# andrewjong/SwapNet

Hardware: AMD Instinct MI355X
Metric: images/sec full G+D step, warp-stage 256x256 bs=32/GPU (higher is better)
Workload: dtype f32; 1 GPU; warp-stage G+D optimize_parameters step, 256x256, bs 32/GPU, fp32 storage and accumulation, GEMM products on the 16-bit MFMA pipe from operand splits: forward / input-gradient GEMMs as 2 fp16 planes of amax-scaled operands (22 of 24 mantissa bits, 3 of 4 terms, the dropped one below 2^-22), weight-gradient GEMMs in the same two-plane form, train mode (dropout 0.5), WarpModule 137.6M + PatchGAN 2.8; step_form=eager launches, global_batch=32, parallelism=dp1

## Files before the change

### include/swapnet_hip.h

```cpp
#ifndef SWAPNET_HIP_H
#define SWAPNET_HIP_H

#include <stddef.h>
#include <stdint.h>

#ifdef __cplusplus
extern "C" {
#endif

typedef struct swn_ctx swn_ctx;
typedef struct swn_model swn_model;

int swn_abi_version(void);
const char* swn_last_error(void);
int swn_is_device_build(void);

int swn_ctx_create(int device, void* hip_stream, int create_stream, size_t workspace_bytes, swn_ctx** out);
int swn_ctx_destroy(swn_ctx* ctx);
int swn_ctx_set_overlap(swn_ctx* ctx, int on);
int swn_ctx_set_patchgan_layers(swn_ctx* ctx, int n_layers);
int swn_ctx_set_patchgan_norm(swn_ctx* ctx, int kind);
int swn_ctx_sync(swn_ctx* ctx);
int swn_ctx_bytes_allocated(swn_ctx* ctx, size_t* out);

int swn_prof_enable(int on);
int swn_prof_reset(void);
int swn_prof_report(char* buf, int len);
int swn_probe_mfma(swn_ctx* ctx, int zeros, int iters, float* out4);
int swn_route_trace(int on);
int swn_route_report(char* buf, int len);
int swn_slot_audit(int on);

int swn_warp_model_create(swn_ctx* ctx, int batch, int height, int width, int is_train, float dropout,
                          swn_model** out);
int swn_texture_model_create(swn_ctx* ctx, int batch, int height, int width, int is_train, int num_roi,
                             swn_model** out);
int swn_warp_model_create_ex(swn_ctx* ctx, int batch, int height, int width, int is_train, float dropout,
                             int body_channels, int cloth_channels, swn_model** out);
int swn_texture_model_create_ex(swn_ctx* ctx, int batch, int height, int width, int is_train, int num_roi,
                                int cloth_channels, swn_model** out);
int swn_texture_model_create_netG(swn_ctx* ctx, int batch, int height, int width, int is_train, int num_roi,
                                  int cloth_channels, int netG, swn_model** out);
int swn_model_create_shared(swn_model* sharer, int batch, int height, int width, swn_model** out);
int swn_model_destroy(swn_model* m);

typedef struct swn_hyper {
  float lr, d_lr, weight_decay, d_weight_decay, b1, b2;
  float lambda_gan, lambda_ce, lambda_l1, lambda_content, lambda_style;
  int gan_mode;
  int warp_mode_ce;
  float grad_scale;
  float d_b1, d_b2;
  int gp_mode;
  float lambda_gp;
} swn_hyper;
int swn_model_set_hyper(swn_model* m, const swn_hyper* h);

int swn_model_param_count(swn_model* m, int net, int* out);
int swn_model_param_info(swn_model* m, int net, int index, char* name, int name_len, int shape[4], int* ndim);
int swn_model_param_set(swn_model* m, int net, int which, const char* name, const float* dev_src);
int swn_model_param_get(swn_model* m, int net, int which, const char* name, float* dev_dst);
int swn_model_optim_step_get(swn_model* m, int net, int* step);
int swn_model_optim_step_set(swn_model* m, int net, int step);
int swn_model_set_optimizer(swn_model* m, int net, int kind, float final_lr, float base_lr, float gamma);

int swn_model_set_input(swn_model* m, int slot, const float* dev_nchw, int n, int c, int h, int w);
int swn_model_set_input_labels(swn_model* m, int slot, const int32_t* dev_labels, int n, int h, int w);
int swn_model_set_input_texture_batch(swn_model* m, const uint8_t* img, int b, int hs, int ws, const uint8_t* labels, int hl, int wl,
                                      const float* rois_raw, int r, const float* sample, const float* mean3, const float* std3,
                                      int x_min, int y_min);
int swn_model_set_input_texture_sources(swn_model* m, const uint8_t* src, size_t src_bytes, const int64_t* geom_host, int b, int hs, int ws,
                                        const uint8_t* labels, int hl, int wl, const float* rois_raw, int r, const float* sample,
                                        const float* mean3, const float* std3, int x_min, int y_min);
int swn_model_set_input_warp_batch(swn_model* m, const uint8_t* body, int b, int hb, int wb, const uint8_t* in_labels,
                                   const uint8_t* tgt_labels, int hl, int wl, const double* maps, int nmaps, const float* mean3,
                                   const float* std3, int load_size, int x_min, int y_min);
int swn_model_set_input_warp_batch_ex(swn_model* m, const uint8_t* body, int b, int hb, int wb, const uint8_t* in_labels,
                                      const uint8_t* tgt_labels, int hl, int wl, const double* maps, int nmaps, const float* mean3,
                                      const float* std3, int load_size, int x_min, int y_min, int flags);
int swn_model_get_output(swn_model* m, int slot, float* dev_nchw);
int swn_model_get_tap(swn_model* m, int net, const char* name, float* dev_nchw, int shape[4]);

int swn_model_get_tap_grad(swn_model* m, int net, const char* name, float* dev_nchw, int shape[4]);

int swn_model_dropout_sites(swn_model* m, int net, int* count);
int swn_model_act_sites(swn_model* m, int net, int* count);
int swn_model_act_pattern(swn_model* m, int net, int site, uint8_t* dev_nchw, int shape[4], int* kind);
int swn_model_dropout_mask(swn_model* m, int net, int site, uint64_t dropout_seed, float* dev_nchw, int shape[4],
                           float* p);

typedef struct swn_pipeline swn_pipeline;
int swn_pipeline_create(swn_model* warp, swn_model* texture, swn_pipeline** out);
int swn_pipeline_destroy(swn_pipeline* p);
int swn_pipeline_run(swn_pipeline* p, int use_graph, int* graph_replayed);
int swn_pipeline_labels(swn_pipeline* p, int32_t** dev_labels);
int swn_pipeline_enable_images(swn_pipeline* p, const float* body_mean3, const float* body_std3, const float* tex_mean3,
                               const float* tex_std3, const uint8_t* colours, int width, int reference_quirk);
int swn_pipeline_images(swn_pipeline* p, uint8_t** dev, int* k);
int swn_pipeline_enable_png(swn_pipeline* p, int rows_per_chunk);
int swn_pipeline_png(swn_pipeline* p, uint8_t** streams, uint32_t** sizes, size_t* stride, int* k);

int swn_model_set_style_context(swn_model* m, const float* all_out_nchw, const float* all_tgt_nchw, int n_total, int n0);
int swn_model_set_gp_random(swn_model* m, const float* alpha_dev, const float* beta_nchw_dev);
int swn_model_discriminate(swn_model* m, const float* x_nchw, float* pred_nchw);
// ... 12 lines not shown
int swn_model_backward_G_part(swn_model* m, float label_real, int part, size_t* ready_off, size_t* ready_count);
int swn_model_optimizer_step(swn_model* m, int net);
int swn_model_optimizer_step_range(swn_model* m, int net, size_t off, size_t count, int first);
int swn_model_step(swn_model* m, const float labels[3], int training, uint64_t dropout_seed);
typedef int (*swn_allreduce_fn)(const void* sendbuf, void* recvbuf, size_t count, int dtype, int op, void* comm, void* stream);
int swn_ctx_attach_comm(swn_ctx* ctx, swn_allreduce_fn fn, void* comm, int world_size);
int swn_model_step_dp(swn_model* m, const float labels[3], int training, uint64_t dropout_seed, int after_forward);
int swn_model_step_captured(swn_model* m, const float labels[3], int training, uint64_t dropout_seed);
int swn_model_get_losses(swn_model* m, float* host_out, int n);

int swn_model_grad_arena(swn_model* m, int net, float** dev_ptr, size_t* count);
int swn_model_weight_arena(swn_model* m, int net, float** dev_ptr, size_t* count);
int swn_model_arena(swn_model* m, int net, int which, float** dev_ptr, size_t* count);

int swn_op_roi_align(swn_ctx* ctx, const float* tex, int b, int c, int h, int w, const float* rois, int r,
                     int ph, int pw, float* out);
int swn_op_roi_align_indices(swn_ctx* ctx, const float* rois, int k, int h, int w, int ph, int pw, int32_t* idx,
                             uint8_t* valid);
int swn_op_decode_labels(swn_ctx* ctx, const float* x, int b, int c, int h, int w, uint8_t* rgb);
int swn_op_image_u8(swn_ctx* ctx, const float* x, int b, int c, int h, int w, const int32_t* labels, int source, const float* rows,
                    int scale_each, int range, const float* rois, int r, const uint8_t* colours, int width, uint8_t* out);
int swn_op_png_encode(swn_ctx* ctx, const uint8_t* img, int n, int h, int w, int rows_per_chunk, uint8_t* streams, size_t stream_stride,
                      uint32_t* sizes);
int swn_png_stream_bound(int h, int w, int rows_per_chunk, size_t* out);
int swn_op_argmax_labels(swn_ctx* ctx, const float* x, int b, int c, int h, int w, int32_t* labels);
int swn_op_labels_to_onehot(swn_ctx* ctx, const int32_t* labels, int b, int c, int h, int w, float* out);
int swn_op_conv(swn_ctx* ctx, int kind, int transposed, int what, int naive, float* x, int n, int ci, int h, int w,
                float* wgt, int co, const float* bias, int act, float* y);
int swn_op_conv_produced(swn_ctx* ctx, int kind, int transposed, int what, int naive, float* x, int n, int ci, int h, int w,
                         float* wgt, int co, const float* bias, int act, float* y, int pre, int post, float* x_out, float* x_slot,
                         float* y_slot, float* z_slot, float* dy_out, float* dy_slot, int* kscale_out);
int swn_op_instance_norm_act(swn_ctx* ctx, const float* x, int n, int c, int h, int w, int act, float* y);
int swn_op_instance_norm_act_bwd(swn_ctx* ctx, const float* x, const float* dy, int n, int c, int h, int w, int act,
                                 float* dx);
int swn_op_batch_norm_act(swn_ctx* ctx, const float* x, int n, int c, int h, int w, int groups, int act, int training,
                          const float* weight, const float* bias, float* running_mean, float* running_var,
                          int64_t* num_batches_tracked, float* y, float* save_stats);
int swn_op_batch_norm_act_bwd(swn_ctx* ctx, const float* x, const float* dy, int n, int c, int h, int w, int groups, int act,
                              const float* weight, const float* bias, float* dx, float* dweight, float* dbias);
int swn_op_batch_norm_act_dropout(swn_ctx* ctx, const float* x, const float* dy, int n, int c, int h, int w, int act, float p,
                                  uint64_t seed, const float* weight, const float* bias, float* y, float* mask, float* dx,
                                  float* dweight, float* dbias);
int swn_op_norm_act_time(swn_ctx* ctx, int kind, int what, const float* x, const float* dy, int n, int c, int h, int w, int groups,
                         int act, int warmup, int iters, float* ms_out);
int swn_op_affine_gather(swn_ctx* ctx, const float* src, float* dst, int b, int c, int h, int w, const double* maps,
                         int nmaps);
int swn_op_chain_resample(swn_ctx* ctx, const float* src, float* dst, int b, int c, int h, int w, const double* maps,
                          int nmaps);
int swn_op_texture_batch(swn_ctx* ctx, const uint8_t* img, int b, int hs, int ws, const uint8_t* labels, int hl, int wl,
                         const float* rois_raw, int r, const float* sample, const float* mean3, const float* std3, int x_min,
                         int y_min, int h, int w, int cloth_channels, float* in_nchw, float* tgt_nchw, float* cloths_nchw,
                         float* rois_out);
int swn_op_resize_u8(swn_ctx* ctx, const uint8_t* src, size_t src_bytes, const int64_t* geom_host, int b, int hs, int ws, uint8_t* dst);
int swn_op_warp_batch(swn_ctx* ctx, const uint8_t* body, int b, int hb, int wb, const uint8_t* in_labels, const uint8_t* tgt_labels, int hl,
                      int wl, const double* maps, int nmaps, const float* mean3, const float* std3, int load_size, int x_min, int y_min,
                      int h, int w, int cloth_channels, float* bodys_nchw, float* input_cloths_nchw, float* target_cloths_nchw);
int swn_op_warp_batch_ex(swn_ctx* ctx, const uint8_t* body, int b, int hb, int wb, const uint8_t* in_labels, const uint8_t* tgt_labels, int hl,
                         int wl, const double* maps, int nmaps, const float* mean3, const float* std3, int load_size, int x_min, int y_min,
                         int h, int w, int cloth_channels, float* bodys_nchw, float* input_cloths_nchw, float* target_cloths_nchw,
                         int flags);
int swn_op_gan_loss(swn_ctx* ctx, int gan_mode, const float* pred, int n, int c, int h, int w, float label,
                    int target_is_real, float grad_scale, float* loss_out, float* dpred);
int swn_op_loss(swn_ctx* ctx, int kind, const float* a_nchw, const float* b_nchw, int n, int c, int h, int w, int pad_c,
                float scale, int accumulate, int n0, int nloc, float* loss_out, float* da_nchw, float* pad_out);
int swn_op_bias_grad(swn_ctx* ctx, const float* dy_nchw, int n, int c, int h, int w, int pad_c, float* db);
int swn_op_norm_act_dropout(swn_ctx* ctx, const float* x, const float* dy, int n, int c, int h, int w, int norm, int act,
                            float p, uint64_t seed, float* y, float* mask, float* dx);
int swn_op_norm_act_bwd2(swn_ctx* ctx, const float* x, const float* gy, const float* u, int n, int c, int h, int w, int act,
                         float* uy, float* ax);
int swn_op_batch_norm_act_bwd2(swn_ctx* ctx, const float* x, const float* gy, const float* u, const float* gamma, const float* beta,
                               int n, int c, int h, int w, int act, float* uy, float* ax, float* dgamma);
int swn_op_norm_act(swn_ctx* ctx, const float* x, const float* dy, const float* residual, int n, int c, int h, int w, int norm,
                    int act, float drop_p, uint64_t seed, int seed_on_device, uint64_t salt, const double* partial_in,
                    int partial_chunks, const int* lead_pad, int want_colsum, float* y, float* stats, float* y_slot, float* dx,
                    float* dx_slot, double* colsum, int* colsum_emitted, float* db, float* y_buf, float* dx_buf);
int swn_op_elementwise(swn_ctx* ctx, int op, const float* a, const float* b, int n, int c, int h, int w, int act, int accumulate,
                       float alpha, float shift, const int* lead_pad, float* out, float* slot, float* out_buf);
int swn_op_resample(swn_ctx* ctx, int op, const float* a, const float* b, int n, int c, int h, int w, int factor, int accumulate,
                    const int* lead_pad, float* out, float* slot, uint8_t* pattern, float* out_buf);
int swn_op_conv_views(swn_ctx* ctx, int kind, int transposed, int what, int naive, float* x, int n, int ci, int h, int w, float* wgt,
                      int co, const float* bias, int act, float* y, const int* views, const int32_t* cimap, int cimap_len,
                      int x_is_input, int dgrad_C, int operand_slots, const float* dx_old, const int* pre_range, float* y_fwd,
                      float* y_slot, float* dw_rows, float* x_buf, float* xg_buf, float* y_buf, float* yg_buf);
int swn_op_adamw(swn_ctx* ctx, float* p, const float* g, float* m, float* v, size_t n, float lr, float b1, float b2,
                 float eps, float wd, int step);
int swn_op_adabound(swn_ctx* ctx, float* p, const float* g, float* m, float* v, size_t n, float lr, float b1, float b2,
                    float eps, float wd, float final_lr, float base_lr, float gamma, int step);

#ifdef __cplusplus
}
#endif
#endif
```

### swapnet_amd/_C.py

```python
import ctypes as C
import os

_HERE = os.path.dirname(os.path.abspath(__file__))
LIB_PATH = os.path.join(_HERE, "csrc", "libswapnet_hip.so")

LOSS_NAMES = ("D", "D_real", "D_fake", "G", "G_gan", "G_ce", "G_l1", "G_content", "G_style", "D_gp")


class SwnHyper(C.Structure):
    _fields_ = [(n, C.c_float) for n in ("lr", "d_lr", "weight_decay", "d_weight_decay", "b1", "b2",
                                         "lambda_gan", "lambda_ce", "lambda_l1", "lambda_content",
                                         "lambda_style")] + [("gan_mode", C.c_int), ("warp_mode_ce", C.c_int), ("grad_scale", C.c_float),
                                                                           ("d_b1", C.c_float), ("d_b2", C.c_float),
                                                                           ("gp_mode", C.c_int), ("lambda_gp", C.c_float)]


class SwapnetHipError(RuntimeError):
    pass


_vp, _fp, _i, _f = C.c_void_p, C.c_void_p, C.c_int, C.c_float

_PROTOS = {
    "swn_abi_version": ([], _i),
    "swn_is_device_build": ([], _i),
    "swn_ctx_create": ([_i, _vp, _i, C.c_size_t, C.POINTER(_vp)], _i),
    "swn_ctx_destroy": ([_vp], _i),
    "swn_ctx_sync": ([_vp], _i),
    "swn_ctx_set_overlap": ([_vp, _i], _i),
    "swn_ctx_set_patchgan_layers": ([_vp, _i], _i),
    "swn_ctx_set_patchgan_norm": ([_vp, _i], _i),
    "swn_ctx_bytes_allocated": ([_vp, C.POINTER(C.c_size_t)], _i),
    "swn_prof_enable": ([_i], _i),
    "swn_prof_reset": ([], _i),
    "swn_prof_report": ([C.c_char_p, _i], _i),
    "swn_probe_mfma": ([_vp, _i, _i, C.POINTER(C.c_float)], _i),
    "swn_route_trace": ([_i], _i),
    "swn_route_report": ([C.c_char_p, _i], _i),
    "swn_slot_audit": ([_i], _i),
    "swn_warp_model_create": ([_vp, _i, _i, _i, _i, _f, C.POINTER(_vp)], _i),
    "swn_texture_model_create": ([_vp, _i, _i, _i, _i, _i, C.POINTER(_vp)], _i),
    "swn_warp_model_create_ex": ([_vp, _i, _i, _i, _i, _f, _i, _i, C.POINTER(_vp)], _i),
    "swn_texture_model_create_ex": ([_vp, _i, _i, _i, _i, _i, _i, C.POINTER(_vp)], _i),
    "swn_texture_model_create_netG": ([_vp, _i, _i, _i, _i, _i, _i, _i, C.POINTER(_vp)], _i),
    "swn_model_create_shared": ([_vp, _i, _i, _i, C.POINTER(_vp)], _i),
    "swn_model_destroy": ([_vp], _i),
    "swn_model_set_hyper": ([_vp, C.POINTER(SwnHyper)], _i),
    "swn_model_param_count": ([_vp, _i, C.POINTER(_i)], _i),
    "swn_model_param_info": ([_vp, _i, _i, C.c_char_p, _i, C.POINTER(_i * 4), C.POINTER(_i)], _i),
    "swn_model_param_set": ([_vp, _i, _i, C.c_char_p, _fp], _i),
    "swn_model_param_get": ([_vp, _i, _i, C.c_char_p, _fp], _i),
    "swn_model_optim_step_get": ([_vp, _i, C.POINTER(_i)], _i),
    "swn_model_optim_step_set": ([_vp, _i, _i], _i),
    "swn_model_set_optimizer": ([_vp, _i, _i, _f, _f, _f], _i),
    "swn_model_set_input": ([_vp, _i, _fp, _i, _i, _i, _i], _i),
    "swn_model_set_input_labels": ([_vp, _i, _vp, _i, _i, _i], _i),
    "swn_model_set_input_texture_batch": ([_vp, _vp, _i, _i, _i, _vp, _i, _i, _fp, _i, _fp, C.POINTER(_f), C.POINTER(_f), _i, _i], _i),
    "swn_model_set_input_texture_sources": ([_vp, _vp, C.c_size_t, _vp, _i, _i, _i, _vp, _i, _i, _fp, _i, _fp, C.POINTER(_f), C.POINTER(_f),
                                             _i, _i], _i),
    "swn_model_set_input_warp_batch": ([_vp, _vp, _i, _i, _i, _vp, _vp, _i, _i, _vp, _i, C.POINTER(_f), C.POINTER(_f), _i, _i, _i], _i),
    "swn_model_set_input_warp_batch_ex": ([_vp, _vp, _i, _i, _i, _vp, _vp, _i, _i, _vp, _i, C.POINTER(_f), C.POINTER(_f), _i, _i, _i, _i], _i),
    "swn_model_get_output": ([_vp, _i, _fp], _i),
    "swn_model_get_tap": ([_vp, _i, C.c_char_p, _fp, C.POINTER(_i * 4)], _i),
    "swn_model_get_tap_grad": ([_vp, _i, C.c_char_p, _fp, C.POINTER(_i * 4)], _i),
    "swn_model_dropout_sites": ([_vp, _i, C.POINTER(_i)], _i),
    "swn_model_act_sites": ([_vp, _i, C.POINTER(_i)], _i),
    "swn_model_act_pattern": ([_vp, _i, _i, _vp, C.POINTER(_i * 4), C.POINTER(_i)], _i),
    "swn_model_dropout_mask": ([_vp, _i, _i, C.c_uint64, _fp, C.POINTER(_i * 4), C.POINTER(_f)], _i),
    "swn_pipeline_create": ([_vp, _vp, C.POINTER(_vp)], _i),
    "swn_pipeline_destroy": ([_vp], _i),
    "swn_pipeline_run": ([_vp, _i, C.POINTER(_i)], _i),
    "swn_pipeline_labels": ([_vp, C.POINTER(_vp)], _i),
    "swn_pipeline_enable_images": ([_vp, C.POINTER(_f), C.POINTER(_f), C.POINTER(_f), C.POINTER(_f), C.POINTER(C.c_uint8), _i, _i], _i),
    "swn_pipeline_images": ([_vp, C.POINTER(_vp), C.POINTER(_i)], _i),
    "swn_pipeline_enable_png": ([_vp, _i], _i),
    "swn_pipeline_png": ([_vp, C.POINTER(_vp), C.POINTER(_vp), C.POINTER(C.c_size_t), C.POINTER(_i)], _i),
    "swn_op_png_encode": ([_vp, _vp, _i, _i, _i, _i, _vp, C.c_size_t, _vp], _i),
    "swn_png_stream_bound": ([_i, _i, _i, C.POINTER(C.c_size_t)], _i),
    "swn_op_image_u8": ([_vp, _fp, _i, _i, _i, _i, _vp, _i, _fp, _i, _i, _fp, _i, _vp, _i, _vp], _i),
    "swn_model_set_style_context": ([_vp, _fp, _fp, _i, _i], _i),
    "swn_model_set_gp_random": ([_vp, _fp, _fp], _i),
    "swn_model_discriminate": ([_vp, _fp, _fp], _i),
    "swn_model_set_discriminate_mode": ([_vp, _i], _i),
    "swn_model_buffer_count": ([_vp, _i, C.POINTER(_i)], _i),
    "swn_model_buffer_info": ([_vp, _i, _i, C.c_char_p, _i, C.POINTER(_i), C.POINTER(_i)], _i),
    "swn_model_buffer_set": ([_vp, _i, C.c_char_p, _vp], _i),
    "swn_model_buffer_get": ([_vp, _i, C.c_char_p, _vp], _i),
    "swn_model_perceptual": ([_vp, _fp, _fp, _i, _fp, _f, _f, _fp], _i),
    "swn_model_forward": ([_vp, _i, C.c_uint64], _i),
    "swn_model_backward_D": ([_vp, _f, _f], _i),
    "swn_model_backward_G": ([_vp, _f], _i),
    "swn_model_backward_G_parts": ([_vp, C.POINTER(C.c_int)], _i),
    "swn_model_backward_G_part": ([_vp, _f, _i, C.POINTER(C.c_size_t), C.POINTER(C.c_size_t)], _i),
    "swn_model_optimizer_step": ([_vp, _i], _i),
    "swn_model_optimizer_step_range": ([_vp, _i, C.c_size_t, C.c_size_t, _i], _i),
    "swn_model_step": ([_vp, C.POINTER(_f * 3), _i, C.c_uint64], _i),
    "swn_model_step_captured": ([_vp, C.POINTER(_f * 3), _i, C.c_uint64], _i),
    "swn_model_step_dp": ([_vp, C.POINTER(_f * 3), _i, C.c_uint64, _i], _i),
    "swn_ctx_attach_comm": ([_vp, _vp, _vp, _i], _i),
    "swn_model_get_losses": ([_vp, C.POINTER(_f), _i], _i),
    "swn_model_grad_arena": ([_vp, _i, C.POINTER(_vp), C.POINTER(C.c_size_t)], _i),
    "swn_model_weight_arena": ([_vp, _i, C.POINTER(_vp), C.POINTER(C.c_size_t)], _i),
    "swn_model_arena": ([_vp, _i, _i, C.POINTER(_vp), C.POINTER(C.c_size_t)], _i),
    "swn_op_roi_align": ([_vp, _fp, _i, _i, _i, _i, _fp, _i, _i, _i, _fp], _i),
    "swn_op_roi_align_indices": ([_vp, _fp, _i, _i, _i, _i, _i, _vp, _vp], _i),
    "swn_op_decode_labels": ([_vp, _fp, _i, _i, _i, _i, _vp], _i),
    "swn_op_argmax_labels": ([_vp, _fp, _i, _i, _i, _i, _vp], _i),
    "swn_op_labels_to_onehot": ([_vp, _vp, _i, _i, _i, _i, _fp], _i),
    "swn_op_conv": ([_vp, _i, _i, _i, _i, _fp, _i, _i, _i, _i, _fp, _i, _fp, _i, _fp], _i),
    "swn_op_conv_produced": ([_vp, _i, _i, _i, _i, _fp, _i, _i, _i, _i, _fp, _i, _fp, _i, _fp, _i, _i, _fp, _fp, _fp, _fp, _fp, _fp, _vp], _i),
    "swn_op_instance_norm_act": ([_vp, _fp, _i, _i, _i, _i, _i, _fp], _i),
    "swn_op_instance_norm_act_bwd": ([_vp, _fp, _fp, _i, _i, _i, _i, _i, _fp], _i),
    "swn_op_batch_norm_act": ([_vp, _fp, _i, _i, _i, _i, _i, _i, _i, _fp, _fp, _fp, _fp, _vp, _fp, _fp], _i),
    "swn_op_batch_norm_act_bwd": ([_vp, _fp, _fp, _i, _i, _i, _i, _i, _i, _fp, _fp, _fp, _fp, _fp], _i),
    "swn_op_batch_norm_act_dropout": ([_vp, _fp, _fp, _i, _i, _i, _i, _i, _f, C.c_uint64, _fp, _fp, _fp, _fp, _fp, _fp, _fp], _i),
    "swn_op_norm_act_time": ([_vp, _i, _i, _fp, _fp, _i, _i, _i, _i, _i, _i, _i, _i, C.POINTER(C.c_float)], _i),
    "swn_op_affine_gather": ([_vp, _fp, _fp, _i, _i, _i, _i, _vp, _i], _i),
    "swn_op_texture_batch": ([_vp, _vp, _i, _i, _i, _vp, _i, _i, _fp, _i, _fp, C.POINTER(_f), C.POINTER(_f), _i, _i, _i, _i, _i,
                             _fp, _fp, _fp, _fp], _i),
    "swn_op_resize_u8": ([_vp, _vp, C.c_size_t, _vp, _i, _i, _i, _vp], _i),
    "swn_op_warp_batch": ([_vp, _vp, _i, _i, _i, _vp, _vp, _i, _i, _vp, _i, C.POINTER(_f), C.POINTER(_f), _i, _i, _i, _i, _i, _i,
                          _fp, _fp, _fp], _i),
    "swn_op_warp_batch_ex": ([_vp, _vp, _i, _i, _i, _vp, _vp, _i, _i, _vp, _i, C.POINTER(_f), C.POINTER(_f), _i, _i, _i, _i, _i, _i,
                             _fp, _fp, _fp, _i], _i),
    "swn_op_chain_resample": ([_vp, _fp, _fp, _i, _i, _i, _i, _vp, _i], _i),
    "swn_op_gan_loss": ([_vp, _i, _fp, _i, _i, _i, _i, _f, _i, _f, _fp, _fp], _i),
    "swn_op_loss": ([_vp, _i, _fp, _fp, _i, _i, _i, _i, _i, _f, _i, _i, _i, _fp, _fp, _fp], _i),
    "swn_op_bias_grad": ([_vp, _fp, _i, _i, _i, _i, _i, _fp], _i),
    "swn_op_norm_act": ([_vp, _fp, _fp, _fp, _i, _i, _i, _i, _i, _i, _f, C.c_uint64, _i, C.c_uint64, _vp, _i, C.POINTER(_i), _i,
                         _fp, _fp, _fp, _fp, _fp, _vp, C.POINTER(_i), _fp, _fp, _fp], _i),
    "swn_op_elementwise": ([_vp, _i, _fp, _fp, _i, _i, _i, _i, _i, _i, _f, _f, C.POINTER(_i), _fp, _fp, _fp], _i),
    "swn_op_resample": ([_vp, _i, _fp, _fp, _i, _i, _i, _i, _i, _i, C.POINTER(_i), _fp, _fp, _vp, _fp], _i),
    "swn_op_conv_views": ([_vp, _i, _i, _i, _i, _fp, _i, _i, _i, _i, _fp, _i, _fp, _i, _fp, C.POINTER(_i), C.POINTER(C.c_int32), _i, _i, _i, _i,
                           _fp, C.POINTER(_i), _fp, _fp, _fp, _fp, _fp, _fp, _fp], _i),
    "swn_op_norm_act_bwd2": ([_vp, _fp, _fp, _fp, _i, _i, _i, _i, _i, _fp, _fp], _i),
    "swn_op_batch_norm_act_bwd2": ([_vp, _fp, _fp, _fp, _fp, _fp, _i, _i, _i, _i, _i, _fp, _fp, _fp], _i),
    "swn_op_norm_act_dropout": ([_vp, _fp, _fp, _i, _i, _i, _i, _i, _i, _f, C.c_uint64, _fp, _fp, _fp], _i),
    "swn_op_adamw": ([_vp, _fp, _fp, _fp, _fp, C.c_size_t, _f, _f, _f, _f, _f, _i], _i),
    "swn_op_adabound": ([_vp, _fp, _fp, _fp, _fp, C.c_size_t, _f, _f, _f, _f, _f, _f, _f, _f, _i], _i),
}


class Lib:

    def __init__(self, path=None):
        self.path = path or LIB_PATH
        if not os.path.exists(self.path):
            raise SwapnetHipError(
                f"{self.path} not found: build it with `python -m swapnet_amd.build` "
                "(hipcc --offload-arch=gfx950).  swapnet_amd has no CPU fallback.")
        import torch
        self.dll = C.CDLL(self.path)
        self.dll.swn_last_error.restype = C.c_char_p
        self.dll.swn_last_error.argtypes = []
        for name, (args, res) in _PROTOS.items():
            fn = getattr(self.dll, name)
            fn.argtypes = args
            fn.restype = res
        self.is_device = bool(self.dll.swn_is_device_build())

    def last_error(self):
        return (self.dll.swn_last_error() or b"").decode()

    def call(self, name, *args):
        rc = getattr(self.dll, name)(*args)
        if rc != 0:
            msg = self.last_error()
            if "not implemented" in msg or "not recognized" in msg:
                raise NotImplementedError(msg)
            if rc == 1:
                raise ValueError(msg)
            raise SwapnetHipError(msg)
        return rc

    @staticmethod
    def exported_symbols():
        return ["swn_last_error"] + list(_PROTOS)


_default = None


def lib():
    global _default
    if _default is None:
        _default = Lib()
        if not _default.is_device:
            raise SwapnetHipError("libswapnet_hip.so is not a device build")
    return _default


def ptr(t):
    if t is None:
        return None
    assert t.is_contiguous(), "tensor must be contiguous"
    return C.c_void_p(t.data_ptr())
```

### swapnet_amd/csrc/capi.cpp

```cpp
#include <algorithm>
#include <cstring>
#include <memory>
#include <string>
#include <vector>

#include "../../include/swapnet_hip.h"
#include <cstdlib>

#include "engine.h"

using namespace swn;

struct CtxBox {
  std::unique_ptr<Ctx> c;
  void* owned_stream = nullptr;
  ~CtxBox() { c.reset(); if (owned_stream) stream_destroy(owned_stream); }
};
struct swn_ctx {
  std::shared_ptr<CtxBox> box;
  Ctx* c = nullptr;
};
struct swn_model {
  std::shared_ptr<CtxBox> keep;
  std::shared_ptr<Model> sharer;
// ... 3 lines not shown
  float dropout = 0.5f;
};
struct swn_pipeline {
  std::shared_ptr<CtxBox> keep;
  std::unique_ptr<Pipeline> p;
};

static thread_local std::string g_err;

template <typename F>
static int guard(F f) {
  try {
    f();
    return 0;
  } catch (const Error& e) {
    g_err = e.what();
    return e.code ? e.code : 1;
  } catch (const std::exception& e) {
    g_err = e.what();
    return 1;
  } catch (...) {
    g_err = "unknown error";
    return 1;
  }
}
#define REQUIRE(cond, msg) \
  do { if (!(cond)) throw Error(1, msg); } while (0)

extern "C" {

int swn_abi_version(void) { return 9; }
const char* swn_last_error(void) { return g_err.c_str(); }
int swn_is_device_build(void) { return is_device_build(); }

int swn_ctx_create(int device, void* hip_stream, int create_stream, size_t workspace_bytes, swn_ctx** out) {
  return guard([&] {
    REQUIRE(out, "swn_ctx_create: out is NULL");
    auto h = std::make_unique<swn_ctx>();
    h->box = std::make_shared<CtxBox>();
    void* st = hip_stream;
    if (create_stream) { st = stream_create(device); h->box->owned_stream = st; }
    else device_check(device);
    if (workspace_bytes < (size_t)64 << 20) workspace_bytes = (size_t)64 << 20;
    h->box->c = std::make_unique<Ctx>(st, workspace_bytes);
    h->c = h->box->c.get();
    h->c->device_index = device;
    if (env_on(getenv("SWN_OVERLAP"))) h->c->enable_side(device);
    *out = h.release();
  });
}
int swn_ctx_destroy(swn_ctx* ctx) {
  return guard([&] {
    if (!ctx) return;
    delete ctx;
  });
}
int swn_ctx_set_overlap(swn_ctx* ctx, int on) {
  return guard([&] {
    REQUIRE(ctx, "ctx is NULL");
    ctx->c->join_side();
    stream_sync(ctx->c->s);
    ctx->c->side_enabled = on != 0;
  });
}
int swn_ctx_attach_comm(swn_ctx* ctx, swn_allreduce_fn fn, void* comm, int world_size) {
  return guard([&] {
    REQUIRE(ctx, "ctx is NULL");
    ctx->c->join_side();
    ctx->c->attach_comm(reinterpret_cast<Ctx::AllReduceFn>(fn), comm, fn ? world_size : 1);
  });
}
int swn_ctx_set_patchgan_layers(swn_ctx* ctx, int n_layers) {
  return guard([&] {
    REQUIRE(ctx, "ctx is NULL");
    REQUIRE(n_layers >= 0 && n_layers <= 5, "n_layers_D must be in [1, 5], or 0 for the 1x1 PixelDiscriminator");
    ctx->c->patchgan_layers = n_layers;
  });
}
int swn_ctx_set_patchgan_norm(swn_ctx* ctx, int kind) {
  return guard([&] {
    REQUIRE(ctx, "ctx is NULL");
    REQUIRE(kind >= 0 && kind <= 2, "normalization layer is not found (0 instance, 1 batch, 2 none)");
    ctx->c->patchgan_norm = kind;
  });
}
int swn_ctx_sync(swn_ctx* ctx) {
  return guard([&] { REQUIRE(ctx, "ctx is NULL"); stream_sync(ctx->c->s); });
}
int swn_ctx_bytes_allocated(swn_ctx* ctx, size_t* out) {
  return guard([&] { REQUIRE(ctx && out, "NULL argument"); *out = ctx->c->bytes_allocated; });
}

int swn_prof_enable(int on) { return guard([&] { prof_enable(on); }); }
int swn_prof_reset(void) { return guard([&] { prof_reset(); }); }
int swn_prof_report(char* buf, int len) { return prof_report(buf, len); }
int swn_probe_mfma(swn_ctx* ctx, int zeros, int iters, float* out4) {
  return guard([&] {
    REQUIRE(ctx && out4, "swn_probe_mfma: NULL argument");
    REQUIRE(iters >= 1 && iters <= (1 << 20), "swn_probe_mfma: iters out of range");
    probe_mfma(ctx->c->s, zeros, iters, out4);
  });
}
int swn_route_trace(int on) { return guard([&] { route_enable(on); }); }
int swn_route_report(char* buf, int len) { return route_report(buf, len); }
int swn_slot_audit(int on) { return guard([&] { slot_audit(on); }); }
struct AuditSuspend {
  int was = slot_audit_on();
  AuditSuspend() { slot_audit(0); }
  ~AuditSuspend() { slot_audit(was); }
};

int swn_warp_model_create_ex(swn_ctx* ctx, int batch, int height, int width, int is_train, float dropout,
                             int body_channels, int cloth_channels, swn_model** out) {
  return guard([&] {
    REQUIRE(ctx && out, "NULL argument");
    REQUIRE(batch > 0 && height > 0 && width > 0, "bad shape");
    auto h = std::make_unique<swn_model>();
    h->keep = ctx->box;
    h->m.reset(create_warp_model(*ctx->c, batch, height, width, is_train != 0, dropout, body_channels, cloth_channels));
    h->kind = 0; h->is_train = is_train != 0; h->dropout = dropout; h->body_channels = body_channels; h->cloth_channels = cloth_channels;
    h->patchgan_layers = ctx->c->patchgan_layers; h->patchgan_norm = ctx->c->patchgan_norm;
    *out = h.release();
  });
}
int swn_warp_model_create(swn_ctx* ctx, int batch, int height, int width, int is_train, float dropout,
                          swn_model** out) {
  return swn_warp_model_create_ex(ctx, batch, height, width, is_train, dropout, 3, 19, out);
}
int swn_texture_model_create_netG(swn_ctx* ctx, int batch, int height, int width, int is_train, int num_roi,
                                  int cloth_channels, int netG, swn_model** out) {
  return guard([&] {
    REQUIRE(ctx && out, "NULL argument");
    auto h = std::make_unique<swn_model>();
    h->keep = ctx->box;
    h->m.reset(create_texture_model(*ctx->c, batch, height, width, is_train != 0, num_roi, cloth_channels, nullptr, netG));
    h->kind = 1; h->is_train = is_train != 0; h->num_roi = num_roi; h->cloth_channels = cloth_channels;
    h->patchgan_layers = ctx->c->patchgan_layers; h->netG = netG;
    *out = h.release();
  });
}
int swn_texture_model_create_ex(swn_ctx* ctx, int batch, int height, int width, int is_train, int num_roi,
                                int cloth_channels, swn_model** out) {
  return swn_texture_model_create_netG(ctx, batch, height, width, is_train, num_roi, cloth_channels, NETG_SWAPNET, out);
}
int swn_texture_model_create(swn_ctx* ctx, int batch, int height, int width, int is_train, int num_roi,
                             swn_model** out) {
  return swn_texture_model_create_ex(ctx, batch, height, width, is_train, num_roi, 19, out);
}
int swn_model_create_shared(swn_model* sharer, int batch, int height, int width, swn_model** out) {
  return guard([&] {
    REQUIRE(sharer && out, "NULL argument");
    REQUIRE(batch > 0 && height > 0 && width > 0, "bad shape");
    std::shared_ptr<Model> root = sharer->sharer ? sharer->sharer : sharer->m;
    Ctx& c = *root->ctx;
    auto h = std::make_unique<swn_model>();
    h->keep = sharer->keep;
    h->sharer = root;
    h->kind = sharer->kind; h->is_train = sharer->is_train; h->dropout = sharer->dropout; h->num_roi = sharer->num_roi;
    h->body_channels = sharer->body_channels; h->cloth_channels = sharer->cloth_channels; h->patchgan_layers = sharer->patchgan_layers;
    h->patchgan_norm = sharer->patchgan_norm; h->netG = sharer->netG;
    const int layers_was = c.patchgan_layers, norm_was = c.patchgan_norm;
    c.patchgan_layers = sharer->patchgan_layers; c.patchgan_norm = sharer->patchgan_norm;
    try {
      if (h->kind == 0)
        h->m.reset(create_warp_model(c, batch, height, width, h->is_train != 0, h->dropout, h->body_channels, h->cloth_channels, root.get()));
      else
// ... 1220 lines not shown
    if (yg_buf) nhwc_to_nchw(s, yo.parent.g, yg_buf, yo.parent.g.C);
    stream_sync(s);
  });
}
int swn_op_norm_act_bwd2(swn_ctx* ctx, const float* x, const float* gy, const float* u, int n, int c, int h, int w, int act,
                         float* uy, float* ax) {
  return guard([&] {
    REQUIRE(ctx && x && gy && u && uy && ax && c % 4 == 0, "bad argument (C must be a multiple of 4)");
    Ctx tmp(ctx->c->s);
    ParamArena A; Net net(tmp, A);
    Var xv = net.alloc_var(n, h, w, c, true), yv = net.alloc_var(n, h, w, c, true), uv = net.alloc_var(n, h, w, c, true);
    net.norm_act(xv, yv, true, act, 0.f);
    net.finalize({});
    nchw_to_nhwc(tmp.s, x, n, c, h, w, xv.v);
    nchw_to_nhwc(tmp.s, gy, n, c, h, w, yv.g);
    nchw_to_nhwc(tmp.s, u, n, c, h, w, uv.v);
    net.forward();
    NormActBwd2Args b2;
    b2.u = uv.v; b2.gy = yv.g; b2.x = xv.v; b2.stats = net.last_stats; b2.uy = uv.g; b2.ax = xv.g; b2.act = act;
    norm_act_bwd2(tmp.s, b2);
    nhwc_to_nchw(tmp.s, uv.g, uy, c);
    nhwc_to_nchw(tmp.s, xv.g, ax, c);
    stream_sync(tmp.s);
  });
}
int swn_op_batch_norm_act_bwd2(swn_ctx* ctx, const float* x, const float* gy, const float* u, const float* gamma, const float* beta,
                               int n, int c, int h, int w, int act, float* uy, float* ax, float* dgamma) {
  return guard([&] {
    REQUIRE(ctx && x && gy && u && gamma && beta && uy && ax && dgamma && c % 4 == 0, "bad argument (C must be a multiple of 4)");
    REQUIRE(n > 0 && c > 0 && h > 0 && w > 0, "bad shape");
    Ctx tmp(ctx->c->s);
    ParamArena A; Net net(tmp, A);
    Var xv = net.alloc_var(n, h, w, c, true), yv = net.alloc_var(n, h, w, c, true), uv = net.alloc_var(n, h, w, c, true);
    float* par = static_cast<float*>(tmp.alloc((size_t)7 * c * sizeof(float)));
    float *gd = par, *bd = par + c, *stats = par + 2 * c, *fold = par + 4 * c, *dg = par + 6 * c;
    dev_copy(tmp.s, gd, gamma, c * sizeof(float));
    dev_copy(tmp.s, bd, beta, c * sizeof(float));
    nchw_to_nhwc(tmp.s, x, n, c, h, w, xv.v);
    nchw_to_nhwc(tmp.s, gy, n, c, h, w, yv.g);
    nchw_to_nhwc(tmp.s, u, n, c, h, w, uv.v);
    BatchNormArgs f;
    f.x = xv.v; f.y = yv.v; f.gamma = gd; f.beta = bd; f.stats = stats; f.fold = fold; f.act = act;
    batch_norm_fwd(tmp.s, f);
    BatchNormBwd2Args b2;
    b2.u = uv.v; b2.gy = yv.g; b2.x = xv.v; b2.stats = stats; b2.fold = fold; b2.gamma = gd;
    b2.uy = uv.g; b2.ax = xv.g; b2.dgamma = dg; b2.act = act;
    batch_norm_bwd2(tmp.s, b2);
    nhwc_to_nchw(tmp.s, uv.g, uy, c);
    nhwc_to_nchw(tmp.s, xv.g, ax, c);
    dev_copy(tmp.s, dgamma, dg, c * sizeof(float));
    stream_sync(tmp.s);
  });
}
int swn_op_norm_act_dropout(swn_ctx* ctx, const float* x, const float* dy, int n, int c, int h, int w, int norm, int act,
                            float p, uint64_t seed, float* y, float* mask, float* dx) {
  return guard([&] {
    REQUIRE(ctx && x && y && c % 4 == 0, "bad argument (C must be a multiple of 4)");
    REQUIRE(p >= 0.f && p < 1.f, "dropout probability must be in [0, 1)");
    Ctx tmp(ctx->c->s);
    ParamArena A; Net net(tmp, A);
    Var xv = net.alloc_var(n, h, w, c, true), yv = net.alloc_var(n, h, w, c, true);
    net.norm_act(xv, yv, norm != 0, act, p);
    net.finalize({});
    net.training = true; net.seed = seed;
    nchw_to_nhwc(tmp.s, x, n, c, h, w, xv.v);
    net.forward();
    nhwc_to_nchw(tmp.s, yv.v, y, c);
    if (mask) {
      if (p > 0.f) {
        const Net::DropSite& d = net.drop_sites.at(0);
        dropout_mask(tmp.s, d.N, d.H, d.W, d.C, d.p, Net::drop_seed(seed, d.salt), mask);
      } else {
        REQUIRE(false, "mask requested with p == 0");
      }
    }
    if (dy && dx) {
      nchw_to_nhwc(tmp.s, dy, n, c, h, w, yv.g);
      net.backward(false, true);
      nhwc_to_nchw(tmp.s, xv.g, dx, c);
    }
    stream_sync(tmp.s);
  });
}
int swn_op_adamw(swn_ctx* ctx, float* p, const float* g, float* m, float* v, size_t n, float lr, float b1, float b2,
                 float eps, float wd, int step) {
  return guard([&] {
    REQUIRE(ctx && p && g && m && v, "NULL argument");
    AdamWArgs a{p, g, m, v, n, lr, b1, b2, eps, wd, step};
    adamw_step(ctx->c->s, a);
    stream_sync(ctx->c->s);
  });
}
int swn_op_adabound(swn_ctx* ctx, float* p, const float* g, float* m, float* v, size_t n, float lr, float b1, float b2,
                    float eps, float wd, float final_lr, float base_lr, float gamma, int step) {
  return guard([&] {
    REQUIRE(ctx && p && g && m && v, "NULL argument");
    REQUIRE(step >= 1 && base_lr > 0.f && gamma > 0.f, "AdaBound needs step >= 1, base_lr > 0, gamma > 0");
    if (!is_device_build()) throw Error(1, "swn_op_adabound: AdaBound is not implemented on the host simulator (HIP kernel only)");
    AdamWArgs a{p, g, m, v, n, lr, b1, b2, eps, wd, step};
    a.kind = OPT_ADABOUND; a.final_lr = final_lr; a.base_lr = base_lr; a.gamma = gamma;
    adamw_step(ctx->c->s, a);
    stream_sync(ctx->c->s);
  });
}

}
```

### swapnet_amd/csrc/engine.cpp

```cpp
#include "engine.h"
#include "png_chunk.h"
#include <memory>

#include <algorithm>
#include <cstddef>
#include <cstdlib>
#include <cstring>
#include <map>
#include <string>
#include <vector>

namespace swn {

namespace {
int g_route = 0;
std::string g_route_label = "-";
char g_route_phase = '-';
std::vector<std::string> g_route_lines;
std::map<std::string, int> g_route_seen;
}
void route_enable(int on) {
  g_route = on;
  if (on) { g_route_lines.clear(); g_route_seen.clear(); g_route_label = "-"; g_route_phase = '-'; }
}
// ... 205 lines not shown
  dg_layout.push_back({op, off});
  return off;
}

namespace {
struct ConvGeom {
  Gather fwd;
  int Ho = 0, Wo = 0;
};
ConvGeom conv_geom(ConvKind kind, int H, int W) {
  ConvGeom c;
  Gather& g = c.fwd;
  switch (kind) {
    case CK_K4S2: g.KH = g.KW = 4; g.stride = 2; g.pad_t = g.pad_l = 1; c.Ho = H / 2; c.Wo = W / 2; break;
    case CK_K3S1_REFLECT: g.KH = g.KW = 3; g.stride = 1; g.pad_t = g.pad_l = 1; g.pad_mode = PAD_REFLECT; c.Ho = H; c.Wo = W; break;
    case CK_K3S1_ZERO: g.KH = g.KW = 3; g.stride = 1; g.pad_t = g.pad_l = 1; c.Ho = H; c.Wo = W; break;
    case CK_K4S1: g.KH = g.KW = 4; g.stride = 1; g.pad_t = g.pad_l = 1; c.Ho = H - 1; c.Wo = W - 1; break;
    case CK_K1S1: g.KH = g.KW = 1; g.stride = 1; g.pad_t = g.pad_l = 0; c.Ho = H; c.Wo = W; break;
    case CK_TAIL_UP:
      g.KH = g.KW = 4; g.stride = 1; g.pad_t = g.pad_l = 2; g.ups = 1; c.Ho = H * 2; c.Wo = W * 2; break;
  }
  g.Ho = c.Ho; g.Wo = c.Wo;
  return c;
}

struct WinoSwitches {
  bool on, s2_on;
  int minc, force_m;
};
WinoSwitches wino_switches() {
  return {env_on(getenv("SWN_WINOGRAD")), env_on(getenv("SWN_WINO_S2")), env_int(getenv("SWN_WINO_MINC"), 0), env_int(getenv("SWN_WINO_M"), 0)};
}

bool s2_wino_wanted(const WinoSwitches& sw, int Cfine, int Ccoarse, int Hc, int Wc) {
  if (!sw.on || !sw.s2_on) return false;
  const int minc = sw.minc > 0 ? sw.minc : 256;
  if (Ccoarse < minc || Cfine < 32 || Cfine % 4 || Ccoarse % 16 || Hc < 2 || Wc < 2) return false;
  if (sw.minc <= 0 && Hc * Wc < 256) return false;
  return (size_t)16 * Cfine * Ccoarse <= ((size_t)1 << 22);
}

int wino_s1_m(const WinoSwitches& sw, ConvKind kind, int Cip, int Co, int H, int W) {
  const bool is_k3 = kind == CK_K3S1_REFLECT || kind == CK_K3S1_ZERO, is_k4 = kind == CK_K4S1;
  const int wm = is_k4 ? 3 : ((sw.force_m != 2 && H % 4 == 0 && W % 4 == 0) ? 4 : 2);
  const int minc = sw.minc > 0 ? sw.minc : (wm == 2 ? 256 : 64);
  const bool wino = sw.on && Cip % 32 == 0 && Co % 32 == 0 && Cip >= minc && Co >= minc && H >= 4 && W >= 4 &&
                    ((is_k3 && H % 2 == 0 && W % 2 == 0) || is_k4);
  return wino ? wm : 0;
}

TView plane_mat(float* p, size_t T, int C) {
  TView v; v.p = p; v.N = 1; v.H = 1; v.W = (int)T; v.C = C; v.cs = C; return v;
}
struct PlaneScale { const int* pair_k = nullptr; const float* amax = nullptr; };
PlaneScale plane_scale(bool pairs, const int* k, const float* amax) { return pairs ? PlaneScale{k, nullptr} : PlaneScale{nullptr, amax}; }
struct PlanePanel { const float* w; const uint16_t* pc; int tile; size_t bs; };
ConvFwdArgs plane_gemm(float* x, float* y, size_t T, int K, int N, int Cout, int P, PlaneScale xs, PlanePanel w) {
  ConvFwdArgs g;
  g.x = plane_mat(x, T, K); g.g.Ho = 1; g.g.Wo = (int)T;
  g.w = w.w; g.Npad = N; g.Cout = Cout;
  g.y = plane_mat(y, T, N);
  g.batch = P; g.x_bs = T * K; g.w_bs = (size_t)K * N; g.y_bs = T * N;
  g.x_pair_k = xs.pair_k; g.x_amax = xs.amax;
  if (w.tile) { g.wpc = w.pc; g.wpc_bn = w.tile; g.wpc_bs = w.bs; }
  return g;
}
ConvWgradArgs plane_wgrad(float* x, float* dy, float* dw, size_t T, int K, int N, int Cout, int P, PlaneScale xs, PlaneScale dys) {
  ConvWgradArgs g;
  g.x = plane_mat(x, T, K); g.g.Ho = 1; g.g.Wo = (int)T;
  g.dy = plane_mat(dy, T, N);
  g.dw = dw; g.Npad = N; g.Cout = Cout;
  g.batch = P; g.x_bs = T * K; g.dy_bs = T * N; g.dw_bs = (size_t)K * N;
  g.x_pair_k = xs.pair_k; g.x_amax = xs.amax;
  g.dy_pair_k = dys.pair_k; g.dy_amax = dys.amax;
  return g;
}

int wino_precut_tile(int xC, int Npad) {
  const int t = conv_precut_tile(xC, Npad);
  return (t == 64 || t == 128) ? t : 0;
}
bool wino_fwd_takes_pairs(int xC, int Npad) { return wino_precut_tile(xC, Npad) != 0 && conv_fwd_takes_pairs(xC, Npad); }

bool bias_on_main() { static const bool on = env_on(getenv("SWN_BIAS_MAIN")); return on; }
}

struct Net::ConvLayer {
  const std::string& name;
  const Var &x, &y;
  ConvKind kind;
  int Ci, Co, Cip, Cop;
  int wi, bi;
  int actf;
  ConvGeom geo;
  bool x_is_input;
  int dgrad_C;
};

void Net::conv(const std::string& name, const Var& x, const Var& y, ConvKind kind, int Ci, int Co, bool bias,
               int actf, const std::vector<int32_t>* cimap, bool x_is_input, int dgrad_C) {
  const WinoSwitches sw = wino_switches();
  const int KH = kind == CK_K1S1 ? 1 : ((kind == CK_K3S1_REFLECT || kind == CK_K3S1_ZERO) ? 3 : 4);
  const ConvGeom geo = conv_geom(kind, x.v.H, x.v.W);
  if (y.v.H != geo.Ho || y.v.W != geo.Wo) throw Error(1, "conv " + name + ": output view has the wrong size");
  const int Cip = x.v.C;
  if (Ci > Cip) throw Error(1, "conv " + name + ": Ci exceeds the input view's channels");
  const int wi = arena.add_weight(name + ".weight", WK_CONV, Co, Ci, KH, KH, Cip, cimap);
  const int bi = bias ? arena.add_bias(name + ".bias", Co) : -1;
  const int Cop = round_up(Co, 4);
  if (y.v.C != Cop) throw Error(1, "conv " + name + ": output view must have round_up(Co,4) channels");
  note_act(actf, y.v);

  auto op = std::make_unique<Op>();
  op->label = name;
  op->param_off = arena.params[wi].off;
  op->reads_net_input = x_is_input;
  const ConvLayer L{name, x, y, kind, Ci, Co, Cip, Cop, wi, bi, actf, geo, x_is_input, dgrad_C};
  if (env_on(getenv("SWN_HEAD_TAPN")) && kind == CK_K4S1 && Co == 1 && Cip % 32 == 0 && actf == ACT_NONE && x.has_grad == y.has_grad)
    conv_head_tapn(L, *op);
  else if (kind == CK_K4S2 && s2_wino && !x_is_input && s2_wino_wanted(sw, Cip, Cop, y.v.H, y.v.W) && Co % 4 == 0)
    conv_wino_s2(L, *op);
  else if (kind == CK_TAIL_UP && sw.on && Cip % 32 == 0 && Cip >= (sw.minc > 0 ? sw.minc : 64) && x.v.H >= 4 && x.v.W >= 4 && Cop <= 32)
    conv_tail_wino(L, *op);
  else if (const int wm = wino_s1_m(sw, kind, Cip, Co, x.v.H, x.v.W))
    conv_wino_s1(L, wm, *op);
  else
    conv_direct(L, *op);
  ops.push_back(std::move(op));
}

void Net::conv_head_tapn(const ConvLayer& L, Op& op) {
  const Var &x = L.x, &y = L.y;
  const int Cip = L.Cip, wi = L.wi, bi = L.bi;
  ParamArena* A = &arena; Op* self = &op;
  const TView xv = x.v, yv = y.v;
  const size_t wt_off = reserve_dg(self, (size_t)Cip * 16), wt2_off = reserve_dg(self, (size_t)16 * Cip);
  const size_t dwt_off = reserve_dg(self, (size_t)Cip * 16);
  note_writer(y.vbase, false);
  Var Z = alloc_var(xv.N, xv.H, xv.W, 16, false);
  const TView zv = Z.v, ygv = y.g, xgv = x.g;
  const bool has_grad = y.has_grad;
  op.repack = [=](Net& n) {
    const ParamDesc& wd = A->params[wi];
    head_pack(n.ctx.s, wd.ws, A->w + wd.off, n.dg + wt_off, n.dg + wt2_off);
  };
  op.fwd = [=](Net& n) {
    n.need(self);
    ConvFwdArgs a;
    a.x = xv; a.g.Ho = xv.H; a.g.Wo = xv.W;
    a.w = n.dg + wt_off; a.Npad = 16; a.Cout = 16; a.y = zv;
    conv_fwd(n.ctx.s, a);
    head_gather(n.ctx.s, zv, bi >= 0 ? A->w + A->params[bi].off : nullptr, yv);
  };
  if (has_grad) op.grad_targets.push_back(x);
  op.bwd = [=](Net& n, Op& me, bool wgrad, bool igrad) {
    if (!has_grad) return;
    const ParamDesc& wd = A->params[wi];
    head_scatter(n.ctx.s, ygv, zv);
    if (wgrad) {
      Stream& sw = n.wgrad_stream();
      ConvWgradArgs wa;
      wa.x = xv; wa.g.Ho = xv.H; wa.g.Wo = xv.W; wa.dy = zv;
      wa.dw = n.dg + dwt_off; wa.Npad = 16; wa.Cout = 16;
      conv_wgrad(sw, wa);
      head_unpack_grad(sw, wd.ws, n.dg + dwt_off, A->g + wd.off);
      if (bi >= 0) n.bias_grad_of(sw, ygv, A->g + A->params[bi].off);
    }
    if (me.reads_net_input && !igrad) return;
    ConvFwdArgs d;
    d.x = zv; d.g.Ho = xv.H; d.g.Wo = xv.W;
    d.w = n.dg + wt2_off; d.Npad = Cip; d.Cout = Cip; d.y = xgv; d.accumulate = me.acc.empty() ? 0 : me.acc[0];
    conv_fwd(n.ctx.s, d);
  };
}

void Net::conv_wino_s2(const ConvLayer& L, Op& op) {
  const Var &x = L.x, &y = L.y;
  const int Co = L.Co, Cip = L.Cip, Cop = L.Cop, wi = L.wi, bi = L.bi, actf = L.actf;
  ParamArena* A = &arena; Op* self = &op;
  const TView xv = x.v, yv = y.v;
  const int sP = 25, sTh = ceil_div(y.v.H, 4), sTw = ceil_div(y.v.W, 4), CV = 4 * Cip;
  const size_t sT = (size_t)x.v.N * sTh * sTw;
  const bool want_dx = x.has_grad && y.has_grad;
  const size_t uf_off = reserve_dg(self, (size_t)sP * CV * Cop);
  const size_t ut_off = want_dx ? reserve_dg(self, (size_t)sP * Cop * CV) : 0;
  float* keepV = (keep_wino_inputs && y.has_grad) ? static_cast<float*>(ctx.alloc(sP * sT * CV * sizeof(float))) : nullptr;
  wsV_need = std::max(wsV_need, sP * sT * (size_t)std::max(CV, Cop));
  wsM_need = std::max(wsM_need, sP * sT * (size_t)std::max(CV, Cop));
  wsU_need = std::max(wsU_need, (size_t)sP * CV * Cop);
  const int pcf = conv_precut_tile(CV, Cop), pct = want_dx ? conv_precut_tile(Cop, CV) : 0;
  const size_t pcf_bs = pcf ? conv_precut_elems(CV, Cop, pcf) : 0, pct_bs = pct ? conv_precut_elems(Cop, CV, pct) : 0;
  const size_t pcf_off = pcf ? reserve_dgp(pcf_bs * sP) : 0, pct_off = pct ? reserve_dgp(pct_bs * sP) : 0;
  const size_t slV = reserve_slot(), slD = reserve_slot();
  note_writer(y.vbase, false);
  const bool pairV_ok = conv_fwd_takes_pairs(CV, Cop) && (!y.has_grad || conv_wgrad_takes_pairs(sT, CV, Cop));
  const bool pairD_ok = conv_wgrad_takes_pairs(sT, CV, Cop) && (!(x.has_grad && y.has_grad) || conv_fwd_takes_pairs(Cop, CV));
  const size_t kV = reserve_k(), kD = reserve_k();
  const float* xbase = x.vbase; const float* ygbase = y.gbase;
  float* keepdM = (y.has_grad && want_dx && share_dy()) ? static_cast<float*>(ctx.alloc(sP * sT * Cop * sizeof(float))) : nullptr;
  op.repack = [=](Net& n) {
    const ParamDesc& wd = A->params[wi];
    const float* wmax = nullptr;
    wino_s2_filter_transform(n.ctx.s, wd.ws, 0, A->w + wd.off, n.dg + uf_off);
    if (pcf) conv_precut(n.ctx.s, n.dg + uf_off, CV, Cop, pcf, sP, (size_t)CV * Cop, n.dgp + pcf_off, &wmax);
    if (want_dx) {
      wino_s2_filter_transform(n.ctx.s, wd.ws, 1, A->w + wd.off, n.dg + ut_off);
      if (pct) conv_precut(n.ctx.s, n.dg + ut_off, Cop, CV, pct, sP, (size_t)Cop * CV, n.dgp + pct_off, &wmax);
    }
  };
  op.fwd = [=](Net& n) {
    n.need(self);
    float* V = keepV ? keepV : n.wsV;
    const float* xin = pairV_ok ? n.slot_if_complete(xbase) : nullptr;
    wino_s2_input_transform(n.ctx.s, xv, sTh, sTw, V, n.amax + slV, xin, n.kscale + kV);
    conv_fwd(n.ctx.s, plane_gemm(V, n.wsM, sT, CV, Cop, Co, sP, plane_scale(xin != nullptr, n.kscale + kV, n.amax + slV),
                                 {n.dg + uf_off, n.dgp + pcf_off, pcf, pcf_bs}));
    wino_output_transform(n.ctx.s, 4, 2, n.wsM, Cop, sTh, sTw, bi >= 0 ? A->w + A->params[bi].off : nullptr, actf, yv, Co, 0);
  };
  Var scratch;
  if (y.has_grad && actf != ACT_NONE) scratch = alloc_var(yv.N, yv.H, yv.W, Cop, false);
  if (want_dx) op.grad_targets.push_back(x);
  const TView ygv = y.g, xgv = x.g, scr = scratch.v;
  const bool has_ygrad = y.has_grad;
  op.bwd = [=](Net& n, Op& me, bool wgrad, bool igrad) {
    if (!has_ygrad) return;
    TView dY = ygv;
    if (actf != ACT_NONE) { act_bwd(n.ctx.s, ygv, yv, scr, actf, 0); dY = scr; }
    const ParamDesc& wd = A->params[wi];
    const bool dx_now = want_dx && !(me.reads_net_input && !igrad);
    const bool shared = keepdM && wgrad && dx_now;
    const float* xin = pairV_ok ? n.slot_if_complete(xbase) : nullptr;
    const float* din = (pairD_ok && actf == ACT_NONE) ? n.slot_if_complete(ygbase) : nullptr;
    const PlaneScale dMs = plane_scale(din != nullptr, n.kscale + kD, n.amax + slD);
    if (shared) wino_dy_transform(n.ctx.s, 4, 2, dY, sTh, sTw, keepdM, n.amax + slD, din, n.kscale + kD);
    if (wgrad) {
      Stream& sw = n.wgrad_stream();
      float* V = keepV ? keepV : n.wsV;
      float* dM = shared ? keepdM : n.wgrad_planes(sw);
      if (!keepV) wino_s2_input_transform(sw, xv, sTh, sTw, V, n.amax + slV, xin, n.kscale + kV);
      if (!shared) wino_dy_transform(sw, 4, 2, dY, sTh, sTw, dM, n.amax + slD, din, n.kscale + kD);
      conv_wgrad(sw, plane_wgrad(V, dM, n.wsU, sT, CV, Cop, Co, sP, plane_scale(xin != nullptr, n.kscale + kV, n.amax + slV), dMs));
      wino_s2_filter_grad(sw, wd.ws, n.wsU, A->g + wd.off);
      if (bi >= 0) n.bias_grad_of(sw, dY, A->g + A->params[bi].off);
    }
    if (!dx_now) return;
    float* dMx = shared ? keepdM : n.wsV;
    if (!shared) wino_dy_transform(n.ctx.s, 4, 2, dY, sTh, sTw, dMx, n.amax + slD, din, n.kscale + kD);
    conv_fwd(n.ctx.s, plane_gemm(dMx, n.wsM, sT, Cop, CV, CV, sP, dMs, {n.dg + ut_off, n.dgp + pct_off, pct, pct_bs}));
    wino_s2_input_adjoint(n.ctx.s, n.wsM, Cip, sTh, sTw, xgv, nullptr, me.acc.empty() ? 0 : me.acc[0]);
  };
}

void Net::conv_tail_wino(const ConvLayer& L, Op& op) {
  const Var &x = L.x, &y = L.y;
  const int Co = L.Co, Cip = L.Cip, Cop = L.Cop, wi = L.wi, bi = L.bi, actf = L.actf;
  ParamArena* A = &arena; Op* self = &op;
  const TView xv = x.v, yv = y.v;
  const ParamDesc wd0 = arena.params[wi];
  const int tP = 36, tTh = ceil_div(x.v.H, 4), tTw = ceil_div(x.v.W, 4), N4 = 4 * Cop;
  const size_t tT = (size_t)x.v.N * tTh * tTw;
  const size_t fe = tail_fold_offset(wd0.ws, 4);
  const size_t fold_off = reserve_dg(self, fe), dfold_off = reserve_dg(self, fe);
  const size_t tu_off = reserve_dg(self, (size_t)tP * Cip * N4);
  float* keepV = (keep_wino_inputs && y.has_grad) ? static_cast<float*>(ctx.alloc(tP * tT * Cip * sizeof(float))) : nullptr;
  wsV_need = std::max(wsV_need, tP * tT * (size_t)std::max(Cip, N4));
  wsM_need = std::max(wsM_need, tP * tT * (size_t)std::max(Cip, N4));
  wsU_need = std::max(wsU_need, (size_t)tP * Cip * N4);
  const int pcu = conv_precut_tile(Cip, N4);
  const size_t pcu_bs = pcu ? conv_precut_elems(Cip, N4, pcu) : 0, pcu_off = pcu ? reserve_dgp(pcu_bs * tP) : 0;
  const size_t slV = reserve_slot(), slD = reserve_slot();
  note_writer(y.vbase, false);
  const bool pairV_ok = conv_fwd_takes_pairs(Cip, N4) && (!y.has_grad || conv_wgrad_takes_pairs(tT, Cip, N4));
  const bool pairD_ok = conv_wgrad_takes_pairs(tT, Cip, N4);
  const size_t kV = reserve_k(), kD = reserve_k();
  const float* xbase = x.vbase;
  const bool want_dx = x.has_grad && y.has_grad;
  const int CopD = (actf != ACT_NONE && want_dx && conv_precut_tile(32, Cip) == 192) ? 32 : Cop;
  const size_t dg_off = want_dx ? reserve_dg(self, dgrad_elems(wd0.ws, 3, CopD, Cip)) : 0;
  const int pc_d = want_dx ? conv_precut_tile(CopD, Cip) : 0;
  const size_t pcd_bs = pc_d ? conv_precut_elems(25 * CopD, Cip, pc_d) : 0, pcd_off = pc_d ? reserve_dgp(pcd_bs) : 0;
  op.repack = [=](Net& n) {
    const ParamDesc& wd = A->params[wi];
    tail_fold_weights(n.ctx.s, wd.ws, A->w + wd.off, n.dg + fold_off);
    tailw_filter_transform(n.ctx.s, wd.ws, n.dg + fold_off, n.dg + tu_off);
    if (pcu) conv_precut(n.ctx.s, n.dg + tu_off, Cip, N4, pcu, tP, (size_t)Cip * N4, n.dgp + pcu_off);
    if (want_dx) {
      repack_dgrad(n.ctx.s, wd.ws, 3, CopD, Cip, A->w + wd.off, n.dg + dg_off);
      if (pc_d) conv_precut(n.ctx.s, n.dg + dg_off, 25 * CopD, Cip, pc_d, 1, 0, n.dgp + pcd_off);
    }
  };
  op.fwd = [=](Net& n) {
    n.need(self);
    float* V = keepV ? keepV : n.wsV;
    const float* xin = pairV_ok ? n.slot_if_complete(xbase) : nullptr;
    wino_input_transform(n.ctx.s, 4, 3, xv, 1, PAD_ZERO, tTh, tTw, V, n.amax + slV, xin, n.kscale + kV);
    conv_fwd(n.ctx.s, plane_gemm(V, n.wsM, tT, Cip, N4, N4, tP, plane_scale(xin != nullptr, n.kscale + kV, n.amax + slV),
                                 {n.dg + tu_off, n.dgp + pcu_off, pcu, pcu_bs}));
    tailw_output_transform(n.ctx.s, n.wsM, tTh, tTw, Cop, bi >= 0 ? A->w + A->params[bi].off : nullptr, actf, yv, Co);
  };
  Var scratch;
  if (y.has_grad && actf != ACT_NONE) scratch = alloc_var(yv.N, yv.H, yv.W, CopD, false);
  if (want_dx) op.grad_targets.push_back(x);
  const TView ygv = y.g, xgv = x.g, scr = CopD != Cop ? scratch.v.slice(0, Cop) : scratch.v, scr_full = scratch.v;
  const bool has_ygrad = y.has_grad;
  const size_t scrSlot = (y.has_grad && actf != ACT_NONE) ? note_writer(scratch.v.p, true) : 0;
  op.bwd = [=](Net& n, Op& me, bool wgrad, bool igrad) {
    if (!has_ygrad) return;
    TView dY = ygv;
    const float* dy_slot = nullptr;
    if (actf != ACT_NONE) { act_bwd(n.ctx.s, ygv, yv, scr, actf, 0, n.amax + scrSlot); dY = scr; dy_slot = n.amax + scrSlot; }
    const ParamDesc& wd = A->params[wi];
    if (wgrad) {
      Stream& sw = n.wgrad_stream();
      float* V = keepV ? keepV : n.wsV;
      float* dM = n.wgrad_planes(sw);
      const float* xin = pairV_ok ? n.slot_if_complete(xbase) : nullptr;
      const float* din = pairD_ok ? dy_slot : nullptr;
      if (!keepV) wino_input_transform(sw, 4, 3, xv, 1, PAD_ZERO, tTh, tTw, V, n.amax + slV, xin, n.kscale + kV);
      tailw_dy_transform(sw, dY, tTh, tTw, Cop, dM, n.amax + slD, din, n.kscale + kD);
      conv_wgrad(sw, plane_wgrad(V, dM, n.wsU, tT, Cip, N4, N4, tP, plane_scale(xin != nullptr, n.kscale + kV, n.amax + slV),
                                 plane_scale(din != nullptr, n.kscale + kD, n.amax + slD)));
      tailw_filter_grad(sw, wd.ws, n.wsU, n.dg + dfold_off);
      tail_unfold_wgrad(sw, wd.ws, n.dg + dfold_off, A->g + wd.off);
      if (bi >= 0) n.bias_grad_of(sw, dY, A->g + A->params[bi].off);
    }
    if (!want_dx || (me.reads_net_input && !igrad)) return;
    ConvFwdArgs d;
    d.x = CopD != Cop ? scr_full : dY;
    d.g.KH = d.g.KW = 5; d.g.stride = 2; d.g.pad_t = d.g.pad_l = 1; d.g.Ho = xv.H; d.g.Wo = xv.W;
    d.w = n.dg + dg_off; d.Npad = Cip; d.Cout = Cip; d.y = xgv; d.accumulate = me.acc.empty() ? 0 : me.acc[0];
    d.x_amax = dy_slot;
// ... 205 lines not shown
        repack_dgrad(n.ctx.s, wd.ws, dg_mode, CopD, Ndg, A->w + wd.off, n.dg + dg_off);
        if (pc_d) conv_precut(n.ctx.s, n.dg + dg_off, dKp, Ndg, pc_d, dpanels, (size_t)dKp * Ndg, n.dgp + pcd_off, &wmax);
      }
      if (folded) tail_fold_weights(n.ctx.s, wd.ws, A->w + wd.off, n.dg + fold_off);
    };
  const TView ygv = y.g, xgv = narrow_dx ? x.g.slice(0, Ndg) : x.g, scr = CopD != Cop ? scratch.v.slice(0, Cop) : scratch.v, scr_full = scratch.v, dxp = dxpad.v;
  const bool has_ygrad = y.has_grad;
  const size_t scrSlot = (y.has_grad && actf != ACT_NONE) ? note_writer(scratch.v.p, true) : 0;
  const float* ygbase = y.gbase;
  op.bwd = [=](Net& n, Op& me, bool wgrad, bool igrad) {
    if (!has_ygrad) return;
    TView dY = ygv;
    const float* dy_slot = nullptr;
    if (actf != ACT_NONE) { act_bwd(n.ctx.s, ygv, yv, scr, actf, 0, n.amax + scrSlot); dY = scr; dy_slot = n.amax + scrSlot; }
    else dy_slot = n.slot_if_complete(ygbase);
    const ParamDesc& wd = A->params[wi];
    const bool dx_now = want_dx && !(me.reads_net_input && !igrad);
    if (wgrad) {
      Stream& sw = n.wgrad_stream();
      ConvWgradArgs wa;
      wa.x = xv; wa.g = gf; wa.dy = dY; wa.dw = A->g + wd.off; wa.Npad = wd.ws.Npad; wa.Cout = Co;
      wa.x_amax = n.slot_if_complete(xbase); wa.dy_amax = dy_slot;
      if (!folded) {
        conv_wgrad(sw, wa);
      } else {
        wa.x_amax = wa.dy_amax = nullptr;
        wa.g = Gather(); wa.g.KH = wa.g.KW = 3; wa.g.stride = 1; wa.g.pad_t = wa.g.pad_l = 1; wa.g.Ho = xv.H; wa.g.Wo = xv.W;
        wa.om.ymul = wa.om.xmul = 2; wa.tail4 = 1;
        wa.dw = n.dg + dfold_off;
        conv_wgrad(sw, wa);
        tail_unfold_wgrad(sw, wd.ws, n.dg + dfold_off, A->g + wd.off);
      }
      if (bi >= 0) n.bias_grad_of((!dx_now && bias_on_main()) ? n.ctx.s : sw, dY, A->g + A->params[bi].off);
    }
    if (!dx_now) return;
    const int accf = me.acc.empty() ? 0 : me.acc[0];
    ConvFwdArgs d;
    d.w = n.dg + dg_off; d.Npad = Ndg; d.Cout = Ndg;
    d.x_amax = dy_slot;
    if (pc_d) { d.wpc = n.dgp + pcd_off; d.wpc_bn = pc_d; d.wpc_bs = pcd_bs; }
    if (kind == CK_K4S2) {
      d.x = dY; d.g.KH = d.g.KW = 2; d.g.stride = 1; d.g.pad_t = 1; d.g.pad_l = 1;
      d.g.Ho = dY.H; d.g.Wo = dY.W;
      d.w_bs = (size_t)4 * Cop * Ndg;
      d.y = xgv; d.om.ymul = 2; d.om.xmul = 2; d.phases = 4; d.accumulate = accf;
      conv_fwd(n.ctx.s, d);
    } else if (kind == CK_K3S1_REFLECT) {
      d.x = dY; d.g = gd; d.y = dxp; d.accumulate = 0;
      conv_fwd(n.ctx.s, d);
      reflect_fold(n.ctx.s, dxp, xgv, accf);
    } else {
      d.x = CopD != Cop ? scr_full : dY; d.g = gd; d.y = xgv; d.accumulate = accf;
      conv_fwd(n.ctx.s, d);
    }
  };
}

void Net::convT(const std::string& name, const Var& x, const Var& y, int Co, bool bias) {
  const WinoSwitches sw = wino_switches();
  if (y.v.H != x.v.H * 2 || y.v.W != x.v.W * 2) throw Error(1, "convT " + name + ": output view has the wrong size");
  const int Cip = x.v.C, Cop = round_up(Co, 4);
  if (y.v.C != Cop) throw Error(1, "convT " + name + ": output view must have round_up(Co,4) channels");
  const int wi = arena.add_weight(name + ".weight", WK_CONVT, Co, Cip, 4, 4, Cip, nullptr);
  const int bi = bias ? arena.add_bias(name + ".bias", Co) : -1;
  auto op = std::make_unique<Op>();
  op->label = name;
  op->param_off = arena.params[wi].off;
  note_writer(y.vbase, false);
  const ConvLayer L{name, x, y, CK_K4S2, Cip, Co, Cip, Cop, wi, bi, ACT_NONE, ConvGeom(), false, 0};
  if (s2_wino && s2_wino_wanted(sw, Cop, Cip, x.v.H, x.v.W) && Co % 4 == 0) convT_wino_s2(L, *op);
  else convT_direct(L, *op);
  ops.push_back(std::move(op));
}

void Net::convT_wino_s2(const ConvLayer& L, Op& op) {
  const Var &x = L.x, &y = L.y;
  const int Cip = L.Cip, Cop = L.Cop, wi = L.wi, bi = L.bi;
  ParamArena* A = &arena; Op* self = &op;
  const TView xv = x.v, yv = y.v, ygv = y.g, xgv = x.g;
  const float* xbase = x.vbase; const float* ygbase = y.gbase;
  const int sP = 25, sTh = ceil_div(x.v.H, 4), sTw = ceil_div(x.v.W, 4), CV = 4 * Cop;
  const size_t sT = (size_t)x.v.N * sTh * sTw;
  const bool want_dx = x.has_grad && y.has_grad;
  const size_t ut_off = reserve_dg(self, (size_t)sP * Cip * CV);
  const size_t uf_off = want_dx ? reserve_dg(self, (size_t)sP * CV * Cip) : 0;
  float* keepM = (keep_wino_inputs && y.has_grad) ? static_cast<float*>(ctx.alloc(sP * sT * Cip * sizeof(float))) : nullptr;
  wsV_need = std::max(wsV_need, sP * sT * (size_t)std::max(CV, Cip));
  wsM_need = std::max(wsM_need, sP * sT * (size_t)std::max(CV, Cip));
  wsU_need = std::max(wsU_need, (size_t)sP * CV * Cip);
  const int pct = conv_precut_tile(Cip, CV), pcf = want_dx ? conv_precut_tile(CV, Cip) : 0;
  const size_t pct_bs = pct ? conv_precut_elems(Cip, CV, pct) : 0, pcf_bs = pcf ? conv_precut_elems(CV, Cip, pcf) : 0;
  const size_t pct_off = pct ? reserve_dgp(pct_bs * sP) : 0, pcf_off = pcf ? reserve_dgp(pcf_bs * sP) : 0;
  const size_t slM = reserve_slot(), slV = reserve_slot();
  const bool wg_pairs = conv_wgrad_takes_pairs(sT, CV, Cip);
  const bool pairM_ok = conv_fwd_takes_pairs(Cip, CV) && (!y.has_grad || wg_pairs);
  const bool pairV_ok = wg_pairs && (!(x.has_grad && y.has_grad) || conv_fwd_takes_pairs(CV, Cip));
  const size_t kM = reserve_k(), kVg = reserve_k();
  float* keepVg = (y.has_grad && want_dx && share_dy()) ? static_cast<float*>(ctx.alloc(sP * sT * CV * sizeof(float))) : nullptr;
  op.repack = [=](Net& n) {
    const ParamDesc& wd = A->params[wi];
    wino_s2_filter_transform(n.ctx.s, wd.ws, 1, A->w + wd.off, n.dg + ut_off);
    const float* wmax = nullptr;
    if (pct) conv_precut(n.ctx.s, n.dg + ut_off, Cip, CV, pct, sP, (size_t)Cip * CV, n.dgp + pct_off, &wmax);
    if (want_dx) {
      wino_s2_filter_transform(n.ctx.s, wd.ws, 0, A->w + wd.off, n.dg + uf_off);
      if (pcf) conv_precut(n.ctx.s, n.dg + uf_off, CV, Cip, pcf, sP, (size_t)CV * Cip, n.dgp + pcf_off, &wmax);
    }
  };
  op.fwd = [=](Net& n) {
    n.need(self);
    float* dM = keepM ? keepM : n.wsV;
    const float* xin = pairM_ok ? n.slot_if_complete(xbase) : nullptr;
    wino_dy_transform(n.ctx.s, 4, 2, xv, sTh, sTw, dM, n.amax + slM, xin, n.kscale + kM);
    conv_fwd(n.ctx.s, plane_gemm(dM, n.wsM, sT, Cip, CV, CV, sP, plane_scale(xin != nullptr, n.kscale + kM, n.amax + slM),
                                 {n.dg + ut_off, n.dgp + pct_off, pct, pct_bs}));
    wino_s2_input_adjoint(n.ctx.s, n.wsM, Cop, sTh, sTw, yv, bi >= 0 ? A->w + A->params[bi].off : nullptr, 0);
  };
  if (want_dx) op.grad_targets.push_back(x);
  const bool has_ygrad = y.has_grad;
  op.bwd = [=](Net& n, Op& me, bool wgrad, bool igrad) {
    if (!has_ygrad) return;
    const ParamDesc& wd = A->params[wi];
    const bool dx_now = want_dx && !(me.reads_net_input && !igrad);
    const bool shared = keepVg && wgrad && dx_now;
    const float* xin = pairM_ok ? n.slot_if_complete(xbase) : nullptr;
    const float* din = pairV_ok ? n.slot_if_complete(ygbase) : nullptr;
    const PlaneScale Vs = plane_scale(din != nullptr, n.kscale + kVg, n.amax + slV);
    if (shared) wino_s2_input_transform(n.ctx.s, ygv, sTh, sTw, keepVg, n.amax + slV, din, n.kscale + kVg);
    if (wgrad) {
      Stream& sw = n.wgrad_stream();
      float* V = shared ? keepVg : n.wgrad_planes(sw);
      float* dM = keepM ? keepM : n.wsV;
      if (!shared) wino_s2_input_transform(sw, ygv, sTh, sTw, V, n.amax + slV, din, n.kscale + kVg);
      if (!keepM) wino_dy_transform(sw, 4, 2, xv, sTh, sTw, dM, n.amax + slM, xin, n.kscale + kM);
      conv_wgrad(sw, plane_wgrad(V, dM, n.wsU, sT, CV, Cip, Cip, sP, Vs, plane_scale(xin != nullptr, n.kscale + kM, n.amax + slM)));
      wino_s2_filter_grad(sw, wd.ws, n.wsU, A->g + wd.off);
      if (bi >= 0) n.bias_grad_of(sw, ygv, A->g + A->params[bi].off);
    }
    if (!dx_now) return;
    float* Vx = shared ? keepVg : n.wsV;
    if (!shared) wino_s2_input_transform(n.ctx.s, ygv, sTh, sTw, Vx, n.amax + slV, din, n.kscale + kVg);
    conv_fwd(n.ctx.s, plane_gemm(Vx, n.wsM, sT, CV, Cip, Cip, sP, Vs, {n.dg + uf_off, n.dgp + pcf_off, pcf, pcf_bs}));
    wino_output_transform(n.ctx.s, 4, 2, n.wsM, Cip, sTh, sTw, nullptr, ACT_NONE, xgv, Cip, me.acc.empty() ? 0 : me.acc[0]);
  };
}

void Net::convT_direct(const ConvLayer& L, Op& op) {
  const Var &x = L.x, &y = L.y;
  const int Co = L.Co, Cip = L.Cip, Cop = L.Cop, wi = L.wi, bi = L.bi;
  ParamArena* A = &arena; Op* self = &op;
  const TView xv = x.v, yv = y.v, ygv = y.g, xgv = x.g;
  const float* xbase = x.vbase; const float* ygbase = y.gbase;
  const size_t phase_elems = (size_t)4 * Cip * round_up(Co, 4);
  const int pc_f = conv_precut_tile(Cip, Cop);
  const size_t pcf_bs = pc_f ? conv_precut_elems(4 * Cip, Cop, pc_f) : 0;
  const size_t pcf_off = pc_f ? reserve_dgp(pcf_bs * 4) : 0;
  op.fwd = [=](Net& n) {
    const ParamDesc& wd = A->params[wi];
    ConvFwdArgs f;
    if (pc_f) { n.need(self); f.wpc = n.dgp + pcf_off; f.wpc_bn = pc_f; f.wpc_bs = pcf_bs; }
    f.x = xv; f.g.KH = f.g.KW = 2; f.g.stride = 1; f.g.pad_t = 1; f.g.pad_l = 1; f.g.Ho = xv.H; f.g.Wo = xv.W;
    f.w = A->w + wd.off; f.w_bs = phase_elems; f.Npad = wd.ws.Npad;
    f.x_amax = n.slot_if_complete(xbase);
    f.bias = bi >= 0 ? A->w + A->params[bi].off : nullptr;
    f.y = yv; f.om.ymul = 2; f.om.xmul = 2; f.phases = 4; f.Cout = Co;
    conv_fwd(n.ctx.s, f);
  };
  const bool want_dx = x.has_grad && y.has_grad;
  size_t dg_off = 0, pcd_off = 0;
  const int pc_d = want_dx ? conv_precut_tile(Cop, Cip) : 0;
  if (want_dx) {
    dg_off = reserve_dg(self, dgrad_elems(arena.params[wi].ws, 2, Cop, Cip));
    if (pc_d) pcd_off = reserve_dgp(conv_precut_elems(16 * Cop, Cip, pc_d));
    op.grad_targets.push_back(x);
  }
  if (want_dx || pc_f)
    op.repack = [=](Net& n) {
      const ParamDesc& wd = A->params[wi];
      const float* wmax = nullptr;
      if (pc_f) conv_precut(n.ctx.s, A->w + wd.off, 4 * Cip, Cop, pc_f, 4, phase_elems, n.dgp + pcf_off, &wmax);
      if (want_dx) {
        repack_dgrad(n.ctx.s, wd.ws, 2, Cop, Cip, A->w + wd.off, n.dg + dg_off);
        if (pc_d) conv_precut(n.ctx.s, n.dg + dg_off, 16 * Cop, Cip, pc_d, 1, 0, n.dgp + pcd_off, &wmax);
      }
    };
  const bool has_ygrad = y.has_grad;
  op.bwd = [=](Net& n, Op& me, bool wgrad, bool igrad) {
    if (!has_ygrad) return;
    const ParamDesc& wd = A->params[wi];
    if (wgrad) {
      ConvWgradArgs wa;
      wa.x = xv; wa.g.KH = wa.g.KW = 2; wa.g.stride = 1; wa.g.pad_t = 1; wa.g.pad_l = 1;
      wa.g.Ho = xv.H; wa.g.Wo = xv.W;
      wa.dy = ygv; wa.om.ymul = 2; wa.om.xmul = 2; wa.phases = 4;
      wa.dw = A->g + wd.off; wa.dw_bs = phase_elems; wa.Npad = wd.ws.Npad; wa.Cout = Co;
      wa.x_amax = n.slot_if_complete(xbase); wa.dy_amax = n.slot_if_complete(ygbase);
      Stream& sw = n.wgrad_stream();
      conv_wgrad(sw, wa);
      if (bi >= 0) n.bias_grad_of(sw, ygv, A->g + A->params[bi].off);
    }
    if (!want_dx || (me.reads_net_input && !igrad)) return;
    ConvFwdArgs d;
    d.x = ygv; d.g.KH = d.g.KW = 4; d.g.stride = 2; d.g.pad_t = d.g.pad_l = 1; d.g.Ho = xv.H; d.g.Wo = xv.W;
    d.w = n.dg + dg_off; d.Npad = Cip; d.Cout = Cip; d.y = xgv; d.accumulate = me.acc.empty() ? 0 : me.acc[0];
    d.x_amax = n.slot_if_complete(ygbase);
    if (pc_d) { d.wpc = n.dgp + pcd_off; d.wpc_bn = pc_d; }
    conv_fwd(n.ctx.s, d);
  };
}

void Net::norm_act(const Var& raw, const Var& y, bool norm, int actf, float drop_p, const Var* residual) {
  auto op = std::make_unique<Op>();
  op->label = "norm_act";
  float* stats = norm ? static_cast<float*>(ctx.alloc((size_t)raw.v.N * raw.v.C * 2 * sizeof(float))) : nullptr;
  last_stats = stats;
  const uint64_t salt = ops.size() + 1;
  if (drop_p > 0.f) drop_sites.push_back({salt, raw.v.N, raw.v.H, raw.v.W, raw.v.C, drop_p});
  if (residual && actf != ACT_NONE) throw Error(1, "norm_act: an activation in front of a residual add is not supported");
  note_act(actf, y.v);
  const TView rv = raw.v, rg = raw.g, yv = y.v, yg = y.g;
  const size_t ySlot = note_writer(y.vbase, true);
  const size_t gSlot = (y.has_grad && raw.has_grad) ? note_writer(raw.gbase, true) : 0;
  const bool has_res = residual != nullptr;
  const Var res = has_res ? *residual : Var();
  const double* partial_in = nullptr;
// ... 892 lines not shown
  auto to_byte = [&](float u) {
    float t;
    if (a.range == RANGE_SIGNED) { volatile float s1 = u + 1.f; volatile float h = s1 / 2.f; volatile float m = h * 255.f; t = m; }
    else { volatile float m = u * 255.f; t = m; }
    return (uint8_t)(int)std::fmin(std::fmax(t, 0.f), 255.f);
  };
  for (int b = 0; b < a.B; ++b) {
    float lo = INFINITY, hi = -INFINITY, den = 1.f;
    if (a.scale_each) {
      for (int p = 0; p < HW; ++p)
        for (int c = 0; c < a.C; ++c) { const float v = a.x.p[((size_t)b * HW + p) * a.x.cs + c]; lo = std::fmin(lo, v); hi = std::fmax(hi, v); }
      den = (float)((double)hi - (double)lo + 1e-5);
    }
    const float* row = a.rows ? a.rows + (size_t)b * (2 * a.C + 1) : nullptr;
    int box[IMAGE_MAX_ROIS][6];
    for (int r = 0; r < a.R; ++r) {
      const float* q = a.rois + ((size_t)b * a.R + r) * 4;
      for (int j = 0; j < 4; ++j) box[r][j] = (int)std::fmin(std::fmax(q[j], -536870912.f), 536870912.f);
      const int s0 = box[r][1] + w, e = box[r][3] - w + 1;
      box[r][4] = s0 <= e ? s0 : e + 1; box[r][5] = s0 <= e ? e - 1 : s0;
    }
    for (int y = 0; y < a.H; ++y)
      for (int x = 0; x < a.W; ++x) {
        const size_t pix = (size_t)b * HW + (size_t)y * a.W + x;
        uint8_t rgb[3] = {0, 0, 0};
        if (a.source == SRC_FLOAT) {
          const float* px = a.x.p + pix * a.x.cs;
          for (int c = 0; c < 3; ++c) {
            const int cc = a.C == 1 ? 0 : c;
            float u = px[cc];
            if (row) {
              volatile float m = u * row[cc];
              volatile float s1 = m + row[a.C + cc];
              u = s1;
              if (row[2 * a.C] != 0.f) u = std::fmin(std::fmax(u, 0.f), 1.f);
            } else if (a.scale_each) {
              volatile float s1 = std::fmin(std::fmax(u, lo), hi) + (-lo);
              volatile float d = s1 / den;
              u = d;
            }
            rgb[c] = to_byte(u);
          }
        } else {
          int best = 0;
          if (a.source == SRC_LABELS) {
            best = a.labels[pix];
          } else {
            const float* px = a.x.p + pix * a.x.cs;
            float m = px[0];
            for (int c = 1; c < a.C; ++c) if (px[c] > m) { m = px[c]; best = c; }
          }
          if (best >= 0 && best < LABEL_PALETTE_SIZE) for (int c = 0; c < 3; ++c) rgb[c] = palette[best][c];
        }
        for (int r = 0; r < a.R; ++r) {
          const int x0 = box[r][0], y0 = box[r][1], x1 = box[r][2], y1 = box[r][3];
          const bool rows_hit = x >= x0 && x <= x1 && ((y >= y0 && y <= y0 + w - 1) || (y >= y1 - w + 1 && y <= y1));
          const bool cols_hit = ((x >= x0 && x <= x0 + w - 1) || (x >= x1 - w + 1 && x <= x1)) && y >= box[r][4] && y <= box[r][5];
          if (rows_hit || cols_hit) for (int c = 0; c < 3; ++c) rgb[c] = a.colours[r * 3 + c];
        }
        for (int c = 0; c < 3; ++c) a.out[pix * 3 + c] = rgb[c];
      }
  }
}

PngGeom png_geometry(int h, int w, int rows_per_chunk) {
  if (h < 1 || w < 1) throw Error(1, "png_encode: empty image");
  if (w > PNG_MAX_WIDTH) throw Error(1, "png_encode: images wider than " + std::to_string(PNG_MAX_WIDTH) + " pixels are refused, got " + std::to_string(w));
  if (h > (1 << 24)) throw Error(1, "png_encode: images of more than 2^24 rows are refused");
  if (rows_per_chunk < 0) throw Error(1, "png_encode: rows_per_chunk must be positive, or 0 for the default");
  const int stride = 1 + 3 * w;
  PngGeom g;
  g.R = rows_per_chunk ? rows_per_chunk : std::max(1, std::min(16, PNG_MAX_CHUNK / stride));
  if ((size_t)g.R * stride > (size_t)PNG_MAX_CHUNK)
    throw Error(1, "png_encode: a chunk of " + std::to_string(g.R) + " rows of " + std::to_string(stride) + " bytes exceeds " +
                       std::to_string(PNG_MAX_CHUNK) + " bytes");
  g.R = std::min(g.R, h);
  g.chunks = (h + g.R - 1) / g.R;
  g.chunk_bytes = g.R * stride;
  g.last_bytes = (h - (g.chunks - 1) * g.R) * stride;
  g.slot = png_slot_stride((size_t)g.chunk_bytes);
  g.bound = 2 + (size_t)(g.chunks - 1) * png_chunk_cap((size_t)g.chunk_bytes) + png_chunk_cap((size_t)g.last_bytes) + 4;
  return g;
}
__attribute__((weak)) void png_encode(Stream&, const PngEncodeArgs&) {
  throw Error(1, "png_encode: PNG encoding is not implemented on the host simulator (HIP kernel only)");
}

}
```

### swapnet_amd/csrc/engine.h

```cpp
#pragma once
#include <cstdlib>
#include <functional>
#include <map>
#include <memory>
#include <string>
#include <vector>

#include "ops.h"

namespace swn {

struct Ctx {
  Stream s;
  Stream side;
  bool has_side = false, side_dirty = false;
  bool side_enabled = true;
  bool use_side() const { return has_side && side_enabled; }
  std::vector<void*> fork_events;
  size_t fork_i = 0;
  void* join_event = nullptr;
  void* owned_side_stream = nullptr;
  void enable_side(int device);
  Stream& fork_side();
  void join_side();
  typedef std::vector<std::pair<void*, size_t>> AllocList;
  AllocList allocs;
  AllocList* sink = nullptr;
  void release(AllocList& list);
  size_t bytes_allocated = 0;
  typedef int (*AllReduceFn)(const void* sendbuf, void* recvbuf, size_t count, int dtype, int op, void* comm, void* stream);
  AllReduceFn comm_fn = nullptr;
  void* comm_handle = nullptr;
  int comm_world = 1;
  int device_index = 0;
  Stream comm_stream;
  void* owned_comm_stream = nullptr;
  std::vector<void*> comm_events;
  size_t comm_ev_i = 0;
  void* comm_join_event = nullptr;
  bool comm_dirty = false;
  void attach_comm(AllReduceFn fn, void* comm, int world);
  Stream& comm_fork();
  void comm_join();
  void all_reduce_sum(Stream& on, float* buf, size_t count);
  int patchgan_layers = 3;
  int patchgan_norm = 0;
  explicit Ctx(void* stream, size_t ws_bytes);
  explicit Ctx(const Stream& shared);
  bool owns_ws = true;
  ~Ctx();
  void* alloc(size_t bytes);
  Ctx(const Ctx&) = delete;
  Ctx& operator=(const Ctx&) = delete;
};

struct AllocScope {
  Ctx& c; Ctx::AllocList* prev;
  AllocScope(Ctx& ctx, Ctx::AllocList& list) : c(ctx), prev(ctx.sink) { c.sink = &list; }
  ~AllocScope() { c.sink = prev; }
  AllocScope(const AllocScope&) = delete;
  AllocScope& operator=(const AllocScope&) = delete;
};

struct Var {
  TView v, g;
  float* vbase = nullptr;
  float* gbase = nullptr;
  bool has_grad = false;
  Var slice(int c0, int c) const;
  Var batch(int n0, int n) const;
};

struct ParamDesc {
  std::string name;
  bool is_bias = false;
  WShape ws{};
  size_t off = 0, elems = 0;
  int n_logical = 0;
  std::vector<int32_t> cimap;
};

struct ParamArena {
  std::vector<ParamDesc> params;
  std::map<std::string, int> index;
  size_t n = 0;
  float *w = nullptr, *g = nullptr, *m = nullptr, *v = nullptr;
  int step = 0;
  int opt_kind = 0;
  float final_lr = 0.1f, base_lr = 0.f, gamma = 1e-3f;
  int version = 1;
  bool frozen = false;
  int add_weight(const std::string& name, int kind, int Co, int Ci, int KH, int KW, int Cip,
                 const std::vector<int32_t>* cimap);
  int add_bias(const std::string& name, int n);
  void allocate(Ctx& c);
  float* base(int which) const { return which == 0 ? w : which == 1 ? g : which == 2 ? m : v; }
};

enum ConvKind { CK_K4S2 = 0, CK_K3S1_REFLECT, CK_K4S1, CK_K3S1_ZERO, CK_TAIL_UP, CK_K1S1  };

class Net;
struct Op {
  std::string label;
  std::function<void(Net&)> fwd;
  std::function<void(Net&, Op&, bool wgrad, bool igrad)> bwd;
  std::vector<Var> grad_targets;
  std::vector<int> acc;
  bool reads_net_input = false;
  size_t param_off = (size_t)-1;
  std::function<void(Net&)> repack;
  void* ready = nullptr;
  bool ready_pending = false;
  int repack_index = -1;
};

class Net {
 public:
  Net(Ctx& c, ParamArena& a) : ctx(c), arena(a) {}
  ~Net() {
    if (refresh_event) event_destroy(refresh_event);
    for (auto& op : ops) if (op->ready) event_destroy(op->ready);
  }
  Ctx& ctx;
  ParamArena& arena;
  std::vector<std::unique_ptr<Op>> ops;
  std::map<std::string, Var> taps;
  bool training = false;
  uint64_t seed = 0;
  const uint64_t* seed_dev = nullptr;
// ... 313 lines not shown
```

### swapnet_amd/csrc/ops.h

```cpp
#pragma once
#include "common.h"
#include <cmath>
#include <cstdlib>
#include <functional>

namespace swn {

struct WShape;

inline bool env_on(const char* v) { return !(v && atoi(v) == 0); }
inline int env_int(const char* v, int dflt) { return v ? atoi(v) : dflt; }

struct Stream {
  void* handle = nullptr;
  char* ws = nullptr;
  size_t ws_bytes = 0;
};

void* event_create();
void event_destroy(void* ev);
void event_record(void* ev, Stream& s);
void stream_wait_event(Stream& s, void* ev);

void* stream_create_current();
// ... 32 lines not shown
struct ConvFwdArgs {
  TView x;
  Gather g;
  const float* w = nullptr;
  int Npad = 0;
  const float* bias = nullptr;
  int act = ACT_NONE;
  int accumulate = 0;
  TView y;
  OutMap om;
  int Cout = 0;
  int batch = 1;
  size_t x_bs = 0, w_bs = 0, y_bs = 0;
  int phases = 0;
  int tail4 = 0;
  const uint16_t* wpc = nullptr;
  int wpc_bn = 0;
  size_t wpc_bs = 0;
  const float* x_amax = nullptr;
  const int* x_pair_k = nullptr;
  float* y_amax = nullptr;
  double* stat_partial = nullptr;
};
int conv_fwd_stat_chunk(int xC, int Npad, int HoWo, int nimg, int K);
constexpr int AMAX_SLOT = 256;
void tensor_amax(Stream& s, const TView& x, float* slot, float floor = 0.f);
void conv_fwd(Stream& s, const ConvFwdArgs& a);
int conv_precut_tile(int xC, int Npad);
size_t conv_precut_elems(int K, int Npad, int bn);
void conv_precut(Stream& s, const float* w, int K, int Npad, int bn, int batch, size_t w_bs, uint16_t* out, const float** amax_io = nullptr);
int conv_precut_planes();
const float* conv_precut_amax(Stream& s, const float* src, size_t rows, int C, int batch, size_t bs);

struct ConvWgradArgs {
  TView x;
  Gather g;
  TView dy;
  OutMap om;
  float* dw = nullptr;
  int Npad = 0;
  int Cout = 0;
  int batch = 1;
  size_t x_bs = 0, dy_bs = 0, dw_bs = 0;
  int phases = 0;
  int tail4 = 0;
  const float* x_amax = nullptr;
  const float* dy_amax = nullptr;
  const int* x_pair_k = nullptr;
  const int* dy_pair_k = nullptr;
};
bool wino_pair_planes();
bool conv_fwd_takes_pairs(int xC, int Npad);
bool conv_wgrad_takes_pairs(size_t T, int K, int Npad);
void conv_wgrad(Stream& s, const ConvWgradArgs& a);

void conv_fwd_naive(Stream& s, const ConvFwdArgs& a);
void conv_wgrad_naive(Stream& s, const ConvWgradArgs& a);

void bias_grad(Stream& s, const TView& dy, float* db);

void reflect_fold(Stream& s, const TView& dxpad, const TView& dx, int accumulate);

void wino_input_transform(Stream& s, int m, int r, const TView& x, int pad, int pad_mode, int Th, int Tw, float* V,
                          float* amax_out = nullptr, const float* in_amax = nullptr, int* kscale_out = nullptr);
void wino_filter_transform(Stream& s, int m, int r, const WShape& w, int mode, const float* packed, float* U);
void wino_filter_transform_pc(Stream& s, int m, int r, const WShape& w, int mode, const float* packed, int bn, uint16_t* out,
                              size_t panel_elems, const float** amax_io = nullptr);
void wino_input_adjoint(Stream& s, int m, int r, float* dV, int C, int pad, int pad_mode, int Th, int Tw, const TView& dx,
                        int accumulate);
void wino_output_transform(Stream& s, int m, int r, const float* M, int Cm, int Th, int Tw, const float* bias, int act,
                           const TView& y, int Cout, int accumulate, float* amax_out = nullptr);
void wino_dy_transform(Stream& s, int m, int r, const TView& dy, int Th, int Tw, float* dM, float* amax_out = nullptr,
                       const float* in_amax = nullptr, int* kscale_out = nullptr);
void tailw_filter_transform(Stream& s, const WShape& w, const float* folded, float* U);
void tailw_filter_grad(Stream& s, const WShape& w, const float* dU, float* dfolded);
void tailw_output_transform(Stream& s, const float* M, int Th, int Tw, int Npad, const float* bias, int act, const TView& y, int Cout);
void tailw_dy_transform(Stream& s, const TView& dy, int Th, int Tw, int Npad, float* dM, float* amax_out = nullptr,
                        const float* in_amax = nullptr, int* kscale_out = nullptr);
void wino_s2_input_transform(Stream& s, const TView& fine, int Th, int Tw, float* V, float* amax_out = nullptr,
                             const float* in_amax = nullptr, int* kscale_out = nullptr);
void wino_s2_input_adjoint(Stream& s, float* dV, int Cf, int Th, int Tw, const TView& fine, const float* bias, int accumulate);
void wino_s2_filter_transform(Stream& s, const WShape& w, int mode, const float* packed, float* U);
void wino_s2_filter_grad(Stream& s, const WShape& w, const float* dU, float* dpacked);
void wino_filter_grad(Stream& s, int m, int r, const WShape& w, const float* dU, float* dpacked);

struct NormActArgs {
  TView x;
  TView y;
  float* stats = nullptr;
  int norm = 1;
  int act = ACT_NONE;
  float drop_p = 0.f;
  uint64_t seed = 0;
  const TView* residual = nullptr;
  float* amax_out = nullptr;
  const uint64_t* seed_base = nullptr;
  uint64_t salt = 0;
  const double* partial_in = nullptr;
  int partial_chunks = 0;
};
void norm_act_fwd(Stream& s, const NormActArgs& a);

struct NormActBwdArgs {
  TView dy;
  TView x;
  const float* stats = nullptr;
  TView dx;
  int norm = 1;
  int act = ACT_NONE;
  float drop_p = 0.f;
  uint64_t seed = 0;
  double* colsum = nullptr;
  float* amax_out = nullptr;
  const uint64_t* seed_base = nullptr;
  uint64_t salt = 0;
};
void norm_act_bwd(Stream& s, const NormActBwdArgs& a);
bool norm_act_bwd_emits_colsum(int HW, int C);
void bias_grad_from_colsums(Stream& s, const double* partial, int N, int C, float* db);

struct BatchNormArgs {
  TView x;
  TView y;
  const float* gamma = nullptr;
  const float* beta = nullptr;
  float* running_mean = nullptr;
  float* running_var = nullptr;
  long long* num_batches_tracked = nullptr;
  float* stats = nullptr;
  float* fold = nullptr;
  int groups = 1;
  int act = ACT_NONE;
  int training = 1;
  float* amax_out = nullptr;
  const double* partial_in = nullptr;
  int partial_chunks = 0;
  float drop_p = 0.f;
  uint64_t seed = 0;
  const uint64_t* seed_base = nullptr;
  uint64_t salt = 0;
};
void batch_norm_fwd(Stream& s, const BatchNormArgs& a);
struct BatchNormBwdArgs {
  TView dy;
  TView x;
  const float* stats = nullptr;
  const float* fold = nullptr;
  TView dx;
  float* dgamma = nullptr;
  float* dbeta = nullptr;
  int groups = 1;
  int act = ACT_NONE;
  float* amax_out = nullptr;
  float drop_p = 0.f;
  uint64_t seed = 0;
  const uint64_t* seed_base = nullptr;
  uint64_t salt = 0;
};
void batch_norm_bwd(Stream& s, const BatchNormBwdArgs& a);
struct BatchNormBwd2Args {
  TView u, gy, x;
  const float* stats = nullptr;
  const float* fold = nullptr;
  const float* gamma = nullptr;
  TView uy, ax;
  float* dgamma = nullptr;
// ... 248 lines not shown
```

### swapnet_amd/csrc/wino.hip

```cpp
#include "hip_util.h"

namespace swn {
namespace {

__device__ __forceinline__ float4 f4add(float4 a, float4 b) { return make_float4(a.x + b.x, a.y + b.y, a.z + b.z, a.w + b.w); }
__device__ __forceinline__ float4 f4sub(float4 a, float4 b) { return make_float4(a.x - b.x, a.y - b.y, a.z - b.z, a.w - b.w); }

__device__ __forceinline__ int wsrc(int e, int ext, int pad_mode) {
  if (pad_mode == PAD_REFLECT) {
    if (e < 0) e = -e;
    else if (e >= ext) e = 2 * ext - 2 - e;
    return e;
  }
  return (e < 0 || e >= ext) ? -1 : e;
}

__global__ __launch_bounds__(256) void wino_input_kernel(const float* x, int xcs, int N, int H, int W, int C, int pad,
                                                         int pad_mode, int Th, int Tw, float* V) {
  const int C4 = C >> 2;
  const size_t T = (size_t)N * Th * Tw;
  const size_t total = T * C4;
  for (size_t i = (size_t)blockIdx.x * 256 + threadIdx.x; i < total; i += (size_t)gridDim.x * 256) {
    const size_t tile = i / C4;
    const int c = (int)(i - tile * C4) * 4;
// ... 604 lines not shown
  const size_t total = T * 4 * C4;
  const int CV = 4 * C;
  float am = 0.f;
  const bool pair = in_amax != nullptr;
  const float psc = pair ? __uint_as_float((unsigned)(127 + pair_scale_exp(in_amax, gain, kscale_out)) << 23) : 1.f;
  for (size_t i = (size_t)blockIdx.x * 256 + threadIdx.x; i < total; i += (size_t)gridDim.x * 256) {
    const int c = (int)(i % C4) * VW; size_t r = i / C4;
    const int q = (int)(r & 3); const size_t tile = r >> 2;
    const int s = q >> 1, t = q & 1;
    const int tx = (int)(tile % Tw); size_t u = tile / Tw;
    const int ty = (int)(u % Th); const int n = (int)(u / Th);
    int sy[A];
#pragma unroll
    for (int a = 0; a < A; ++a) { const int e = 2 * (4 * ty + a) - 1 + s; sy[a] = (e >= 0 && e < H) ? e : -1; }
    vt tt[A][A];
#pragma unroll
    for (int b = 0; b < A; ++b) {
      const int e = 2 * (4 * tx + b) - 1 + t;
      const int sx = (e >= 0 && e < W) ? e : -1;
      vt d[A];
#pragma unroll
      for (int a = 0; a < A; ++a)
        d[a] = (sy[a] >= 0 && sx >= 0) ? *reinterpret_cast<const vt*>(x + ((size_t)(n * H + sy[a]) * W + sx) * xcs + c) : vt(0.f);
#pragma unroll
      for (int rr = 0; rr < A; ++rr) {
        vt acc = vt(0.f);
#pragma unroll
        for (int k = 0; k < A; ++k)
          if (F42::BT[rr][k] != 0.f) acc += F42::BT[rr][k] * d[k];
        tt[rr][b] = acc;
      }
    }
#pragma unroll
    for (int a = 0; a < A; ++a)
#pragma unroll
      for (int j = 0; j < A; ++j) {
        vt acc = vt(0.f);
#pragma unroll
        for (int k = 0; k < A; ++k)
          if (F42::BT[j][k] != 0.f) acc += F42::BT[j][k] * tt[a][k];
        *reinterpret_cast<vt*>(V + ((size_t)(a * A + j) * T + tile) * CV + q * C + c) = pair ? pairv<VW>(acc, psc) : acc;
        am = fmaxf(am, fvamax<VW>(acc));
      }
  }
  if (!pair) amax_fold(am, amax_out);
}

__global__ __launch_bounds__(256) void wino_s2_fold_kernel(const float* P, int C, int N, int H, int W, int Th, int Tw, const float* bias,
                                                           float* dx, int dcs, int accumulate) {
  constexpr int A = 5, M = 4;
  const int C4 = C >> 2, CV = 4 * C;
  const size_t T = (size_t)N * Th * Tw;
  const size_t total = (size_t)N * H * W * C4;
  for (size_t i = (size_t)blockIdx.x * 256 + threadIdx.x; i < total; i += (size_t)gridDim.x * 256) {
    const size_t px = i / C4;
    const int c = (int)(i - px * C4) * 4;
    const int n = (int)(px / ((size_t)H * W));
    const int rem = (int)(px - (size_t)n * H * W);
    const int r = rem / W, cc = rem - r * W;
    const int s = (r + 1) & 1, t = (cc + 1) & 1;
    const int qy = (r + 1 - s) >> 1, qx = (cc + 1 - t) >> 1;
    float4 acc = F4ZERO;
    for (int ty = min(qy / M, Th - 1); ty >= 0 && qy - M * ty < A; --ty) {
      const int a = qy - M * ty;
      for (int tx = min(qx / M, Tw - 1); tx >= 0 && qx - M * tx < A; --tx) {
        const int b = qx - M * tx;
        const size_t tile = ((size_t)n * Th + ty) * Tw + tx;
        acc = f4add(acc, *reinterpret_cast<const float4*>(P + ((size_t)(a * A + b) * T + tile) * CV + (2 * s + t) * C + c));
      }
    }
    if (bias) { acc.x += bias[c]; acc.y += bias[c + 1]; acc.z += bias[c + 2]; acc.w += bias[c + 3]; }
    float* d = dx + px * dcs + c;
    if (accumulate) acc = f4add(acc, *reinterpret_cast<const float4*>(d));
    *reinterpret_cast<float4*>(d) = acc;
  }
}

__device__ __forceinline__ size_t s2_widx(const WShape& w, int kh, int kw, int cf, int cc) {
  if (w.kind == WK_CONV) return ((size_t)(kh * 4 + kw) * w.Cip + cf) * w.Npad + cc;
  const int a = (3 - kh) & 1, dy = (3 - kh - a) >> 1, b = (3 - kw) & 1, dx = (3 - kw - b) >> 1;
  return (size_t)(a * 2 + b) * 4 * w.Cip * w.Npad + ((size_t)(dy * 2 + dx) * w.Cip + cc) * w.Npad + cf;
}

__global__ __launch_bounds__(256) void wino_s2_filter_kernel(WShape w, int mode, int Cf, int Cc, const float* packed, float* U) {
  constexpr int A = 5;
  const size_t total = (size_t)Cf * Cc;
  const size_t i = (size_t)blockIdx.x * 256 + threadIdx.x;
  if (i >= total) return;
  const int cf = mode == 0 ? (int)(i / Cc) : (int)(i % Cf), cc = mode == 0 ? (int)(i % Cc) : (int)(i / Cf);
  const size_t plane = (size_t)4 * Cf * Cc;
#pragma unroll
  for (int q = 0; q < 4; ++q) {
    const int s = q >> 1, t = q & 1;
    float g[2][2];
#pragma unroll
    for (int a = 0; a < 2; ++a)
#pragma unroll
      for (int b = 0; b < 2; ++b) g[a][b] = packed[s2_widx(w, 2 * a + s, 2 * b + t, cf, cc)];
    float tt[A][2];
#pragma unroll
    for (int r = 0; r < A; ++r)
#pragma unroll
      for (int b = 0; b < 2; ++b) tt[r][b] = F42::G[r][0] * g[0][b] + F42::G[r][1] * g[1][b];
    const size_t o = mode == 0 ? ((size_t)(q * Cf + cf) * Cc + cc) : ((size_t)cc * 4 * Cf + q * Cf + cf);
#pragma unroll
    for (int a = 0; a < A; ++a)
#pragma unroll
      for (int j = 0; j < A; ++j) U[(size_t)(a * A + j) * plane + o] = tt[a][0] * F42::G[j][0] + tt[a][1] * F42::G[j][1];
  }
}

__global__ __launch_bounds__(256) void wino_s2_filter_grad_kernel(WShape w, int Cf, int Cc, const float* dU, float* dpacked) {
  constexpr int A = 5;
  const size_t total = (size_t)Cf * Cc;
  const size_t i = (size_t)blockIdx.x * 256 + threadIdx.x;
  if (i >= total) return;
  const int cf = (int)(i / Cc), cc = (int)(i % Cc);
  const size_t plane = (size_t)4 * Cf * Cc;
#pragma unroll
  for (int q = 0; q < 4; ++q) {
    const int s = q >> 1, t = q & 1;
    const size_t o = (size_t)(q * Cf + cf) * Cc + cc;
    float tt[2][A];
#pragma unroll
    for (int b = 0; b < A; ++b) {
      float u[A];
#pragma unroll
      for (int a = 0; a < A; ++a) u[a] = dU[(size_t)(a * A + b) * plane + o];
#pragma unroll
      for (int r = 0; r < 2; ++r) {
        float acc = 0.f;
#pragma unroll
        for (int a = 0; a < A; ++a) f1mac(acc, F42::G[a][r], u[a]);
        tt[r][b] = acc;
      }
    }
#pragma unroll
    for (int a = 0; a < 2; ++a)
#pragma unroll
      for (int b = 0; b < 2; ++b) {
        float acc = 0.f;
#pragma unroll
        for (int k = 0; k < A; ++k) f1mac(acc, F42::G[k][b], tt[a][k]);
        dpacked[s2_widx(w, 2 * a + s, 2 * b + t, cf, cc)] = acc;
      }
  }
}


typedef unsigned wu32x4 __attribute__((ext_vector_type(4)));
__device__ __forceinline__ void cut8_store(const float (&u)[8], wu32x4* o, size_t e0, size_t plane_stride) {
  unsigned hi[4], mid[4], lo[4];
#pragma unroll
  for (int j = 0; j < 4; ++j) {
    const float x0 = u[2 * j], x1 = u[2 * j + 1];
    const unsigned u0 = __float_as_uint(x0), u1 = __float_as_uint(x1);
    const float r0 = x0 - __uint_as_float(u0 & 0xffff0000u), r1 = x1 - __uint_as_float(u1 & 0xffff0000u);
    const unsigned v0 = __float_as_uint(r0), v1 = __float_as_uint(r1);
    const float s0 = r0 - __uint_as_float(v0 & 0xffff0000u), s1 = r1 - __uint_as_float(v1 & 0xffff0000u);
    hi[j] = (u0 >> 16) | (u1 & 0xffff0000u);
    mid[j] = (v0 >> 16) | (v1 & 0xffff0000u);
    lo[j] = (__float_as_uint(s0) >> 16) | (__float_as_uint(s1) & 0xffff0000u);
  }
  o[e0] = wu32x4{hi[0], hi[1], hi[2], hi[3]};
  o[e0 + plane_stride] = wu32x4{mid[0], mid[1], mid[2], mid[3]};
  o[e0 + 2 * plane_stride] = wu32x4{lo[0], lo[1], lo[2], lo[3]};
}

typedef _Float16 wf16x2 __attribute__((ext_vector_type(2)));
__device__ __forceinline__ void cut8_store_h(const float (&u)[8], float sb, wu32x4* o, size_t e0, size_t plane_stride, bool low_plane) {
  unsigned hi[4], lo[4];
#pragma unroll
  for (int j = 0; j < 4; ++j) {
    const float x0 = u[2 * j] * sb, x1 = u[2 * j + 1] * sb;
    const wf16x2 hh = wf16x2{(_Float16)x0, (_Float16)x1};
    hi[j] = __builtin_bit_cast(unsigned, hh);
    lo[j] = __builtin_bit_cast(unsigned, wf16x2{(_Float16)(x0 - (float)hh[0]), (_Float16)(x1 - (float)hh[1])});
  }
  o[e0] = wu32x4{hi[0], hi[1], hi[2], hi[3]};
  if (low_plane) o[e0 + plane_stride] = wu32x4{lo[0], lo[1], lo[2], lo[3]};
}
__device__ __forceinline__ int wino_scale_exp(const float* part, int lane, int top) {
  float m = fmaxf(fmaxf(part[lane], part[lane + 64]), fmaxf(part[lane + 128], part[lane + 192]));
#pragma unroll
  for (int o = 32; o; o >>= 1) m = fmaxf(m, __shfl_xor(m, o));
  if (!(m > 0.f) || m > 3.0e38f) return 0;
  const int e = (int)((__float_as_uint(m) >> 23) & 255u) - 127;
  const int k = top - 1 - e;
  return k < -100 ? -100 : (k > 100 ? 100 : k);
}

template <class F>
__global__ __launch_bounds__(256) void winog_filter_pc_kernel(WShape w, int mode, int K, int Nn, int BN, const float* packed,
                                                              unsigned short* out, size_t panel_elems, const float* wamax, int planes) {
  constexpr int A = F::A, R = F::R;
  const int NBc = BN / 32, tiles_n = (Nn + BN - 1) / BN;
  const size_t total = (size_t)(K / 8) * tiles_n * BN;
  const size_t i = ((size_t)(blockIdx.x / (8 * A)) * 8 + blockIdx.x % 8) * 256 + threadIdx.x;
  const int PL = planes;
  int kB = 0;
  if (wamax) kB = wino_scale_exp(wamax, threadIdx.x & 63, 10);
  if (i >= total) return;
  const int nl = (int)(i % BN); const size_t q = i / BN;
  const int tn = (int)(q % tiles_n), kq = (int)(q / tiles_n);
  const int n = tn * BN + nl;
  const int pos = (nl % NBc) * 32 + nl / NBc;
  const int a = (int)(blockIdx.x % (8 * A)) / 8;
  float Ga[R];
#pragma unroll
  for (int qq = 0; qq < R; ++qq) Ga[qq] = F::G[a][qq];
  float t[8][R];
#pragma unroll
  for (int kk = 0; kk < 8; ++kk)
#pragma unroll
    for (int b = 0; b < R; ++b) t[kk][b] = 0.f;
  if (mode == 0) {
    if (n < w.Npad) {
#pragma unroll
      for (int kk = 0; kk < 8; ++kk) {
        const int k = kq * 8 + kk;
        if (k < w.Cip) {
#pragma unroll
          for (int qq = 0; qq < R; ++qq)
#pragma unroll
            for (int b = 0; b < R; ++b) t[kk][b] += Ga[qq] * packed[((size_t)(qq * R + b) * w.Cip + k) * w.Npad + n];
        }
      }
    }
  } else if (n < w.Cip && kq * 8 < w.Npad) {
#pragma unroll
    for (int qq = 0; qq < R; ++qq)
#pragma unroll
      for (int b = 0; b < R; ++b) {
        const int tap = mode == 1 ? (R - 1 - qq) * R + (R - 1 - b) : qq * R + b;
        const float4* src = reinterpret_cast<const float4*>(packed + ((size_t)tap * w.Cip + n) * w.Npad + kq * 8);
        const float4 g0 = src[0], g1 = src[1];
        t[0][b] += Ga[qq] * g0.x; t[1][b] += Ga[qq] * g0.y; t[2][b] += Ga[qq] * g0.z; t[3][b] += Ga[qq] * g0.w;
        t[4][b] += Ga[qq] * g1.x; t[5][b] += Ga[qq] * g1.y; t[6][b] += Ga[qq] * g1.z; t[7][b] += Ga[qq] * g1.w;
      }
  }
  const size_t e0 = ((((size_t)(kq >> 1) * tiles_n + tn) * 2 + (kq & 1)) * PL) * BN + pos;
  const float sb = __uint_as_float((unsigned)(127 + kB) << 23);
#pragma unroll
  for (int j = 0; j < A; ++j) {
    float u[8];
#pragma unroll
    for (int kk = 0; kk < 8; ++kk) {
      float s = 0.f;
#pragma unroll
      for (int qq = 0; qq < R; ++qq) f1mac(s, F::G[j][qq], t[kk][qq]);
      u[kk] = s;
    }
    unsigned short* panel = out + (size_t)(a * A + j) * panel_elems;
    if (wamax) {
      cut8_store_h(u, sb, reinterpret_cast<wu32x4*>(panel), e0, (size_t)BN, PL == 2);
      if (i == 0) *reinterpret_cast<int*>(panel + (size_t)(K / 16) * tiles_n * 2 * PL * BN * 8) = kB;
    } else {
      cut8_store(u, reinterpret_cast<wu32x4*>(panel), e0, (size_t)BN);
    }
  }
}


__device__ __forceinline__ size_t tailw_fold_off(int Cip, int Npad, int ph) {
  const int pre = ph == 0 ? 0 : (ph == 1 ? 4 : (ph == 2 ? 10 : 16));
  return (size_t)pre * Cip * Npad;
}
__global__ __launch_bounds__(256) void tailw_filter_kernel(int Cip, int Npad, const float* folded, float* U) {
  constexpr int A = 6, R = 3;
  const int N4 = 4 * Npad;
  const size_t total = (size_t)Cip * N4;
  const size_t i = (size_t)blockIdx.x * 256 + threadIdx.x;
  if (i >= total) return;
  const int ci = (int)(i / N4), n = (int)(i % N4);
  const int ph = n / Npad, co = n - ph * Npad, a = ph >> 1, b = ph & 1;
  const float* f = folded + tailw_fold_off(Cip, Npad, ph);
  float g[R][R];
#pragma unroll
  for (int r = 0; r < R; ++r)
#pragma unroll
    for (int c = 0; c < R; ++c) g[r][c] = (r < 2 + a && c < 2 + b) ? f[((size_t)(r * (2 + b) + c) * Cip + ci) * Npad + co] : 0.f;
  float t[A][R];
#pragma unroll
  for (int r = 0; r < A; ++r)
#pragma unroll
    for (int c = 0; c < R; ++c) {
      float s = 0.f;
#pragma unroll
      for (int q = 0; q < R; ++q) f1mac(s, F43::G[r][q], g[q][c]);
      t[r][c] = s;
    }
#pragma unroll
  for (int r = 0; r < A; ++r)
#pragma unroll
    for (int j = 0; j < A; ++j) {
      float s = 0.f;
#pragma unroll
      for (int q = 0; q < R; ++q) f1mac(s, F43::G[j][q], t[r][q]);
      U[(size_t)(r * A + j) * total + i] = s;
    }
}
__global__ __launch_bounds__(256) void tailw_filter_grad_kernel(int Cip, int Npad, const float* dU, float* dfolded) {
  constexpr int A = 6, R = 3;
  const int N4 = 4 * Npad;
  const size_t total = (size_t)Cip * N4;
  const size_t i = (size_t)blockIdx.x * 256 + threadIdx.x;
  if (i >= total) return;
  const int ci = (int)(i / N4), n = (int)(i % N4);
  const int ph = n / Npad, co = n - ph * Npad, a = ph >> 1, b = ph & 1;
  float t[R][A];
#pragma unroll
  for (int j = 0; j < A; ++j) {
    float u[A];
#pragma unroll
    for (int r = 0; r < A; ++r) u[r] = dU[(size_t)(r * A + j) * total + i];
#pragma unroll
    for (int q = 0; q < R; ++q) {
      float s = 0.f;
#pragma unroll
      for (int r = 0; r < A; ++r) f1mac(s, F43::G[r][q], u[r]);
      t[q][j] = s;
    }
  }
  float* f = dfolded + tailw_fold_off(Cip, Npad, ph);
#pragma unroll
  for (int r = 0; r < R; ++r)
#pragma unroll
    for (int c = 0; c < R; ++c) {
      if (r >= 2 + a || c >= 2 + b) continue;
      float s = 0.f;
#pragma unroll
      for (int j = 0; j < A; ++j) f1mac(s, F43::G[j][c], t[r][j]);
      f[((size_t)(r * (2 + b) + c) * Cip + ci) * Npad + co] = s;
    }
}
__global__ __launch_bounds__(256) void tailw_output_kernel(const float* Mx, int N, int Th, int Tw, int Npad, const float* bias, int act,
                                                           float* y, int ycs, int yH, int yW, int Cout) {
  constexpr int A = 6, M = 4;
  const int C4 = Npad >> 2, CM = 4 * Npad;
  const size_t T = (size_t)N * Th * Tw;
  const size_t total = T * 4 * C4;
  for (size_t i = (size_t)blockIdx.x * 256 + threadIdx.x; i < total; i += (size_t)gridDim.x * 256) {
    const int c = (int)(i % C4) * 4; size_t r = i / C4;
    const int ph = (int)(r & 3); const size_t tile = r >> 2;
    const int a = ph >> 1, b = ph & 1;
    const int tx = (int)(tile % Tw); size_t u = tile / Tw;
// ... 5 lines not shown
#pragma unroll
      for (int k = 0; k < A; ++k) m[k] = *reinterpret_cast<const float4*>(Mx + ((size_t)(k * A + j) * T + tile) * CM + ph * Npad + c);
#pragma unroll
      for (int q = 0; q < M; ++q) {
        float4 s = F4ZERO;
#pragma unroll
        for (int k = 0; k < A; ++k) f4mac(s, F43::AT[q][k], m[k]);
        s1[q][j] = s;
      }
    }
    float4 bv = F4ZERO;
    if (bias) bv = make_float4(c < Cout ? bias[c] : 0.f, c + 1 < Cout ? bias[c + 1] : 0.f, c + 2 < Cout ? bias[c + 2] : 0.f,
                               c + 3 < Cout ? bias[c + 3] : 0.f);
#pragma unroll
    for (int q = 0; q < M; ++q)
#pragma unroll
      for (int jj = 0; jj < M; ++jj) {
        const int oy = 2 * (M * ty + q) + a, ox = 2 * (M * tx + jj) + b;
        if (oy >= yH || ox >= yW) continue;
        float4 v = F4ZERO;
#pragma unroll
        for (int k = 0; k < A; ++k) f4mac(v, F43::AT[jj][k], s1[q][k]);
        v = f4add(v, bv);
        v.x = act_apply(v.x, act); v.y = act_apply(v.y, act); v.z = act_apply(v.z, act); v.w = act_apply(v.w, act);
        float* dst = y + ((size_t)(n * yH + oy) * yW + ox) * ycs + c;
        if (c + 3 < Cout) {
          *reinterpret_cast<float4*>(dst) = v;
        } else {
          const float vv[4] = {v.x, v.y, v.z, v.w};
          for (int e = 0; e < 4 && c + e < Cout; ++e) dst[e] = vv[e];
        }
      }
  }
}
__global__ __launch_bounds__(256) void tailw_dy_kernel(const float* dy, int dcs, int N, int yH, int yW, int Th, int Tw, int Npad,
                                                       float* dM, float* amax_out, const float* in_amax, float gain, int* kscale_out) {
  constexpr int A = 6, M = 4;
  const int C4 = Npad >> 2, CM = 4 * Npad;
  const size_t T = (size_t)N * Th * Tw;
  const size_t total = T * 4 * C4;
  float am = 0.f;
  const bool pair = in_amax != nullptr;
  const float psc = pair ? __uint_as_float((unsigned)(127 + pair_scale_exp(in_amax, gain, kscale_out)) << 23) : 1.f;
  for (size_t i = (size_t)blockIdx.x * 256 + threadIdx.x; i < total; i += (size_t)gridDim.x * 256) {
    const int c = (int)(i % C4) * 4; size_t r = i / C4;
    const int ph = (int)(r & 3); const size_t tile = r >> 2;
    const int a = ph >> 1, b = ph & 1;
    const int tx = (int)(tile % Tw); size_t u = tile / Tw;
    const int ty = (int)(u % Th); const int n = (int)(u / Th);
    float4 rr[A][M];
#pragma unroll
    for (int jj = 0; jj < M; ++jj) {
      float4 g[M];
#pragma unroll
      for (int q = 0; q < M; ++q) {
        const int oy = 2 * (M * ty + q) + a, ox = 2 * (M * tx + jj) + b;
        g[q] = (oy < yH && ox < yW) ? *reinterpret_cast<const float4*>(dy + ((size_t)(n * yH + oy) * yW + ox) * dcs + c) : F4ZERO;
      }
#pragma unroll
      for (int p = 0; p < A; ++p) {
        float4 s = F4ZERO;
#pragma unroll
        for (int q = 0; q < M; ++q) f4mac(s, F43::AT[q][p], g[q]);
        rr[p][jj] = s;
      }
    }
#pragma unroll
    for (int p = 0; p < A; ++p)
#pragma unroll
      for (int j = 0; j < A; ++j) {
        float4 s = F4ZERO;
#pragma unroll
        for (int jj = 0; jj < M; ++jj) f4mac(s, F43::AT[jj][j], rr[p][jj]);
        *reinterpret_cast<float4*>(dM + ((size_t)(p * A + j) * T + tile) * CM + ph * Npad + c) = pair ? pair4(s, psc) : s;
        am = fmaxf(am, f4amax(s));
      }
  }
  if (!pair) amax_fold(am, amax_out);
}

inline unsigned wgrid(size_t total) { return (unsigned)std::min<size_t>(std::max<size_t>((total + 255) / 256, 1), 256 * 32); }

}

static int variant(int m, int r) {
  if (m == 2 && r == 3) return 0;
  if (m == 4 && r == 3) return 1;
  if (m == 3 && r == 4) return 2;
  if (m == 4 && r == 2) return 3;
  throw Error(1, "winograd: supported forms are F(2,3), F(4,3), F(3,4) and the strided F(4,2)");
}
static constexpr int wino_vec_width() { return 2; }
static float input_gain(int v) { return v == 3 ? 9.f : 100.f; }
static float dy_gain(int v) { return v == 1 ? 225.f : (v == 2 ? 49.f : 16.f); }
void wino_input_transform(Stream& s, int m, int r, const TView& x, int pad, int pad_mode, int Th, int Tw, float* V, float* amax_out,
                          const float* in_amax, int* kscale_out) {
  const int v = variant(m, r);
  if (v == 3) throw Error(1, "wino_input_transform: F(4,2) is the strided form (wino_s2_input_transform)");
  if (x.C % 4 || x.cs % 4) throw Error(1, "wino_input_transform: C must be a multiple of 4");
  const int vw = wino_vec_width();
  const size_t total = (size_t)x.N * Th * Tw * (x.C / (v == 0 ? 4 : vw));
  const dim3 grid(wgrid(total));
  if (v == 0 && in_amax) throw Error(1, "wino_input_transform: F(2,3) planes have no pair form");
#define SWN_WIN_LAUNCH(F, VW)                                                                                                  \
  hipLaunchKernelGGL((winog_input_kernel<F, VW>), grid, dim3(256), 0, hs(s), x.p, x.cs, x.N, x.H, x.W, x.C, pad, pad_mode, Th, \
                     Tw, V, amax_out, in_amax, input_gain(v), kscale_out)
  if (v == 0)
    hipLaunchKernelGGL(wino_input_kernel, grid, dim3(256), 0, hs(s), x.p, x.cs, x.N, x.H, x.W, x.C, pad, pad_mode, Th, Tw, V);
  else if (v == 1) SWN_WIN_LAUNCH(F43, 2);
  else SWN_WIN_LAUNCH(F34, 2);
#undef SWN_WIN_LAUNCH
  check_launch("wino_input_transform");
  if (in_amax && slot_audit_on()) {
    audit_slot(s, "wino_input_transform", in_amax, x.p, x.pixels(), x.C, (size_t)x.cs, 1, 0);
    audit_pair_planes(s, "wino_input_transform", V, (size_t)(m + r - 1) * (m + r - 1) * x.N * Th * Tw * x.C, kscale_out);
  }
}
void wino_filter_transform(Stream& s, int m, int r, const WShape& w, int mode, const float* packed, float* U) {
  const int v = variant(m, r);
  if (v == 3) throw Error(1, "wino_filter_transform: F(4,2) is the strided form (wino_s2_filter_transform)");
  const int K = mode == 0 ? w.Cip : w.Npad, Nn = mode == 0 ? w.Npad : w.Cip;
  const dim3 grid((unsigned)(((size_t)K * Nn + 255) / 256));
  if (v == 0) hipLaunchKernelGGL(wino_filter_kernel, grid, dim3(256), 0, hs(s), w, mode, K, Nn, packed, U);
  else if (v == 1) hipLaunchKernelGGL(winog_filter_kernel<F43>, grid, dim3(256), 0, hs(s), w, mode, K, Nn, packed, U);
  else hipLaunchKernelGGL(winog_filter_kernel<F34>, grid, dim3(256), 0, hs(s), w, mode, K, Nn, packed, U);
  check_launch("wino_filter_transform");
}
void wino_filter_transform_pc(Stream& s, int m, int r, const WShape& w, int mode, const float* packed, int bn, uint16_t* out,
                              size_t panel_elems, const float** amax_io) {
  const int v = variant(m, r);
  if (v != 1 && v != 2) throw Error(1, "wino_filter_transform_pc: the 6-point forms F(4,3) / F(3,4) only");
  if (mode < 0 || mode > 2) throw Error(1, "wino_filter_transform_pc: mode 0, 1 or 2");
  const int K = mode == 0 ? w.Cip : w.Npad, Nn = mode == 0 ? w.Npad : w.Cip;
  if (K % 16 || (bn != 64 && bn != 128)) throw Error(1, "wino_filter_transform_pc: K must be a multiple of 16, tile 64 or 128");
  const size_t total = (size_t)(K / 8) * ((Nn + bn - 1) / bn) * bn;
  const dim3 grid((unsigned)((((total + 255) / 256 + 7) / 8) * 8) * (unsigned)(m + r - 1));
  const float* wamax = (amax_io && *amax_io) ? *amax_io : conv_precut_amax(s, packed, (size_t)r * r * w.Cip, w.Npad, 1, 0);
  if (amax_io) *amax_io = wamax;
  if (v == 1)
    hipLaunchKernelGGL(winog_filter_pc_kernel<F43>, grid, dim3(256), 0, hs(s), w, mode, K, Nn, bn, packed, out, panel_elems, wamax,
                       conv_precut_planes());
  else
    hipLaunchKernelGGL(winog_filter_pc_kernel<F34>, grid, dim3(256), 0, hs(s), w, mode, K, Nn, bn, packed, out, panel_elems, wamax,
                       conv_precut_planes());
  check_launch("wino_filter_transform_pc");
}
void wino_output_transform(Stream& s, int m, int r, const float* M, int Cm, int Th, int Tw, const float* bias, int act,
                           const TView& y, int Cout, int accumulate, float* amax_out) {
  const int v = variant(m, r);
  if (v == 0 && amax_out) throw Error(1, "wino_output_transform: the F(2,3) kernel has no amax fold");
  const size_t total = (size_t)y.N * Th * Tw * ((Cout + 3) / 4);
  const dim3 grid(wgrid(total));
  if (v == 0)
    hipLaunchKernelGGL(wino_output_kernel, grid, dim3(256), 0, hs(s), M, Cm, y.N, Th, Tw, bias, act, y.p, y.cs, y.H, y.W,
                       Cout, accumulate);
  else if (v == 1)
    hipLaunchKernelGGL(winog_output_kernel<F43>, grid, dim3(256), 0, hs(s), M, Cm, y.N, Th, Tw, bias, act, y.p, y.cs, y.H,
                       y.W, Cout, accumulate, amax_out);
  else if (v == 2)
    hipLaunchKernelGGL(winog_output_kernel<F34>, grid, dim3(256), 0, hs(s), M, Cm, y.N, Th, Tw, bias, act, y.p, y.cs, y.H,
                       y.W, Cout, accumulate, amax_out);
  else
    hipLaunchKernelGGL(winog_output_kernel<F42>, grid, dim3(256), 0, hs(s), M, Cm, y.N, Th, Tw, bias, act, y.p, y.cs, y.H,
                       y.W, Cout, accumulate, amax_out);
  check_launch("wino_output_transform");
}
// ... 5 lines not shown
  const size_t total = (size_t)dy.N * Th * Tw * (dy.C / vw);
  const dim3 grid(wgrid(total));
  if (v == 0 && in_amax) throw Error(1, "wino_dy_transform: F(2,3) planes have no pair form");
#define SWN_WDY_LAUNCH(F, VW)                                                                                                       \
  hipLaunchKernelGGL((winog_dy_kernel<F, VW>), grid, dim3(256), 0, hs(s), dy.p, dy.cs, dy.N, dy.H, dy.W, dy.C, Th, Tw, dM, amax_out, \
                     in_amax, dy_gain(v), kscale_out)
  if (v == 0)
    hipLaunchKernelGGL(wino_dy_kernel, grid, dim3(256), 0, hs(s), dy.p, dy.cs, dy.N, dy.H, dy.W, dy.C, Th, Tw, dM);
  else if (v == 1) SWN_WDY_LAUNCH(F43, 2);
  else if (v == 2) SWN_WDY_LAUNCH(F34, 2);
  else SWN_WDY_LAUNCH(F42, 2);
#undef SWN_WDY_LAUNCH
  check_launch("wino_dy_transform");
  if (in_amax && slot_audit_on()) {
    audit_slot(s, "wino_dy_transform", in_amax, dy.p, dy.pixels(), dy.C, (size_t)dy.cs, 1, 0);
    audit_pair_planes(s, "wino_dy_transform", dM, (size_t)(m + r - 1) * (m + r - 1) * dy.N * Th * Tw * dy.C, kscale_out);
  }
}
void tailw_filter_transform(Stream& s, const WShape& w, const float* folded, float* U) {
  const size_t total = (size_t)w.Cip * 4 * w.Npad;
  hipLaunchKernelGGL(tailw_filter_kernel, dim3((unsigned)((total + 255) / 256)), dim3(256), 0, hs(s), w.Cip, w.Npad, folded, U);
  check_launch("tailw_filter_transform");
}
void tailw_filter_grad(Stream& s, const WShape& w, const float* dU, float* dfolded) {
  const size_t total = (size_t)w.Cip * 4 * w.Npad;
  hipLaunchKernelGGL(tailw_filter_grad_kernel, dim3((unsigned)((total + 255) / 256)), dim3(256), 0, hs(s), w.Cip, w.Npad, dU, dfolded);
  check_launch("tailw_filter_grad");
}
void tailw_output_transform(Stream& s, const float* M, int Th, int Tw, int Npad, const float* bias, int act, const TView& y, int Cout) {
  if (Npad % 4 || y.cs % 4 || y.C < Npad) throw Error(1, "tailw_output_transform: bad channel counts");
  const size_t total = (size_t)y.N * Th * Tw * 4 * (Npad / 4);
  hipLaunchKernelGGL(tailw_output_kernel, dim3(wgrid(total)), dim3(256), 0, hs(s), M, y.N, Th, Tw, Npad, bias, act, y.p, y.cs, y.H, y.W, Cout);
  check_launch("tailw_output_transform");
}
void tailw_dy_transform(Stream& s, const TView& dy, int Th, int Tw, int Npad, float* dM, float* amax_out, const float* in_amax,
                        int* kscale_out) {
  if (Npad % 4 || dy.cs % 4 || dy.C < Npad) throw Error(1, "tailw_dy_transform: bad channel counts");
  const size_t total = (size_t)dy.N * Th * Tw * 4 * (Npad / 4);
  hipLaunchKernelGGL(tailw_dy_kernel, dim3(wgrid(total)), dim3(256), 0, hs(s), dy.p, dy.cs, dy.N, dy.H, dy.W, Th, Tw, Npad, dM, amax_out,
                     in_amax, 225.f, kscale_out);
  check_launch("tailw_dy_transform");
  if (in_amax && slot_audit_on()) {
    audit_slot(s, "tailw_dy_transform", in_amax, dy.p, dy.pixels(), dy.C, (size_t)dy.cs, 1, 0);
    audit_pair_planes(s, "tailw_dy_transform", dM, (size_t)36 * dy.N * Th * Tw * 4 * Npad, kscale_out);
  }
}
void wino_s2_input_transform(Stream& s, const TView& x, int Th, int Tw, float* V, float* amax_out, const float* in_amax, int* kscale_out) {
  if (x.C % 4 || x.cs % 4) throw Error(1, "wino_s2_input_transform: C must be a multiple of 4");
  const int vw = wino_vec_width();
  const size_t total = (size_t)x.N * Th * Tw * 4 * (x.C / vw);
  hipLaunchKernelGGL(wino_s2_input_kernel<2>, dim3(wgrid(total)), dim3(256), 0, hs(s), x.p, x.cs, x.N, x.H, x.W, x.C, Th, Tw, V,
                       amax_out, in_amax, 9.f, kscale_out);
  check_launch("wino_s2_input_transform");
  if (in_amax && slot_audit_on()) {
    audit_slot(s, "wino_s2_input_transform", in_amax, x.p, x.pixels(), x.C, (size_t)x.cs, 1, 0);
    audit_pair_planes(s, "wino_s2_input_transform", V, (size_t)25 * x.N * Th * Tw * 4 * x.C, kscale_out);
  }
}
void wino_s2_input_adjoint(Stream& s, float* dV, int Cf, int Th, int Tw, const TView& dx, const float* bias, int accumulate) {
  if (Cf % 4 || dx.C != Cf || dx.cs % 4) throw Error(1, "wino_s2_input_adjoint: bad channel count");
  const size_t T = (size_t)dx.N * Th * Tw;
  hipLaunchKernelGGL(winog_patch_kernel<F42>, dim3(wgrid(T * Cf)), dim3(256), 0, hs(s), dV, 4 * Cf, T);
  hipLaunchKernelGGL(wino_s2_fold_kernel, dim3(wgrid(dx.pixels() * (Cf / 4))), dim3(256), 0, hs(s), dV, Cf, dx.N, dx.H, dx.W, Th, Tw,
                     bias, dx.p, dx.cs, accumulate);
  check_launch("wino_s2_input_adjoint");
}
static void s2_dims(const WShape& w, int& Cf, int& Cc) {
  if (w.KH != 4 || w.KW != 4) throw Error(1, "strided Winograd: k4 s2 layers only");
  Cf = w.kind == WK_CONV ? w.Cip : w.Npad;
  Cc = w.kind == WK_CONV ? w.Npad : w.Cip;
}
void wino_s2_filter_transform(Stream& s, const WShape& w, int mode, const float* packed, float* U) {
  int Cf, Cc;
  s2_dims(w, Cf, Cc);
  hipLaunchKernelGGL(wino_s2_filter_kernel, dim3((unsigned)(((size_t)Cf * Cc + 255) / 256)), dim3(256), 0, hs(s), w, mode, Cf, Cc, packed, U);
  check_launch("wino_s2_filter_transform");
}
void wino_s2_filter_grad(Stream& s, const WShape& w, const float* dU, float* dpacked) {
  int Cf, Cc;
  s2_dims(w, Cf, Cc);
  hipLaunchKernelGGL(wino_s2_filter_grad_kernel, dim3((unsigned)(((size_t)Cf * Cc + 255) / 256)), dim3(256), 0, hs(s), w, Cf, Cc, dU, dpacked);
  check_launch("wino_s2_filter_grad");
}
void wino_input_adjoint(Stream& s, int m, int r, float* dV, int C, int pad, int pad_mode, int Th, int Tw, const TView& dx,
                        int accumulate) {
  const int v = variant(m, r);
  if (v == 3) throw Error(1, "wino_input_adjoint: F(4,2) is the strided form (wino_s2_input_adjoint)");
  if (C % 4 || dx.C != C || dx.cs % 4) throw Error(1, "wino_input_adjoint: bad channel count");
  const size_t T = (size_t)dx.N * Th * Tw;
  const dim3 grid(wgrid(T * (C / 4)));
  if (v == 0) hipLaunchKernelGGL(winog_patch_kernel<F23>, grid, dim3(256), 0, hs(s), dV, C, T);
  else if (v == 1) hipLaunchKernelGGL(winog_patch_kernel<F43>, grid, dim3(256), 0, hs(s), dV, C, T);
  else hipLaunchKernelGGL(winog_patch_kernel<F34>, grid, dim3(256), 0, hs(s), dV, C, T);
  const int A = m + r - 1;
  hipLaunchKernelGGL(wino_fold_kernel, dim3(wgrid(dx.pixels() * (C / 4))), dim3(256), 0, hs(s), dV, C, dx.N, dx.H, dx.W, m, A, pad,
                     pad_mode, Th, Tw, dx.p, dx.cs, accumulate);
  check_launch("wino_input_adjoint");
}
void wino_filter_grad(Stream& s, int m, int r, const WShape& w, const float* dU, float* dpacked) {
  const int v = variant(m, r);
  if (v == 3) throw Error(1, "wino_filter_grad: F(4,2) is the strided form (wino_s2_filter_grad)");
  const size_t total = (size_t)w.Cip * w.Npad;
  const dim3 grid((unsigned)((total + 255) / 256));
  if (v == 0) hipLaunchKernelGGL(wino_filter_grad_kernel, grid, dim3(256), 0, hs(s), w, dU, dpacked);
  else if (v == 1) hipLaunchKernelGGL(winog_filter_grad_kernel<F43>, grid, dim3(256), 0, hs(s), w, dU, dpacked);
  else hipLaunchKernelGGL(winog_filter_grad_kernel<F34>, grid, dim3(256), 0, hs(s), w, dU, dpacked);
  check_launch("wino_filter_grad");
}

}
```

### swapnet_amd/engine.py

```python
import ctypes as C
import os
from collections import OrderedDict

import torch

from . import _C

NET_G, NET_D, NET_VGG = 0, 1, 2
OPT_ADAMW, OPT_ADABOUND = 0, 1
W_WEIGHT, W_GRAD, W_EXP_AVG, W_EXP_AVG_SQ = 0, 1, 2, 3
NORM_KINDS = {"instance": 0, "batch": 1, "none": 2}
NETG_KINDS = {"swapnet": 0, "unet_128": 1}


class Context:

    def __init__(self, device=None, lib=None, workspace_mb=512, use_torch_stream=True):
        self.lib = lib or _C.lib()
        if self.lib.is_device:
            if not torch.cuda.is_available():
                raise _C.SwapnetHipError("no HIP device visible; swapnet_amd has no CPU path")
            self.device = torch.device("cuda", torch.cuda.current_device() if device is None else int(device))
            torch.cuda.set_device(self.device)
            self.torch_stream = torch.cuda.current_stream(self.device)
            stream = C.c_void_p(self.torch_stream.cuda_stream)
            if os.environ.get("SWAPNET_OWN_STREAM") == "1":
                use_torch_stream = False
            dev_index, create = self.device.index, int(not use_torch_stream)
        else:
            self.device = torch.device("cpu")
            stream, dev_index, create = None, 0, 0
        h = C.c_void_p()
        self.lib.call("swn_ctx_create", dev_index, stream, create, C.c_size_t(workspace_mb << 20), C.byref(h))
        self.handle = h
        self.owns_stream = bool(create)
        self._copy_stream = None

    def upload(self, tensor, dtype, key=None):
        t = tensor.detach()
        if self.device.type != "cuda" or t.is_cuda:
            return t.to(device=self.device, dtype=dtype).contiguous(), None
        t = t.to(dtype=dtype).contiguous()
        if self._copy_stream is None:
            self._copy_stream = torch.cuda.Stream(device=self.device)
            self._staging = {}
        cs, main = self._copy_stream, torch.cuda.current_stream(self.device)
        if key is None:
            with torch.cuda.stream(cs):
                d = t.to(self.device, non_blocking=True)
            main.wait_stream(cs)
            d.record_stream(main)
            return d, None
        st = self._staging.setdefault(key, {"bufs": [None, None], "events": [None, None], "i": 0})
        i = st["i"]
        st["i"] ^= 1
        buf = st["bufs"][i]
        if buf is None or buf.shape != t.shape or buf.dtype != dtype:
            buf = torch.empty(t.shape, dtype=dtype, device=self.device)
            st["bufs"][i], st["events"][i] = buf, None
        if st["events"][i] is not None:
            cs.wait_event(st["events"][i])
        with torch.cuda.stream(cs):
            buf.copy_(t, non_blocking=True)
        main.wait_stream(cs)
        return buf, (key, i)

    def consumed(self, token):
        if token is None:
            return
        ev = torch.cuda.Event()
        ev.record(torch.cuda.current_stream(self.device))
        self._staging[token[0]]["events"][token[1]] = ev

    def set_overlap(self, on):
        self.lib.call("swn_ctx_set_overlap", self.handle, int(bool(on)))

    def sync(self):
        self.lib.call("swn_ctx_sync", self.handle)

    def attach_comm(self, fn_ptr, comm, world):
        self.lib.call("swn_ctx_attach_comm", self.handle, C.c_void_p(fn_ptr) if fn_ptr else None,
                      comm if comm is not None else None, int(world))

    def route_trace(self, on):
        self.lib.call("swn_route_trace", int(bool(on)))

    def route_report(self):
        need = self.lib.dll.swn_route_report(None, 0)
        buf = C.create_string_buffer(need + 16)
        self.lib.dll.swn_route_report(buf, need + 16)
        return [l for l in buf.value.decode().split("\n") if l]

    def bytes_allocated(self):
        n = C.c_size_t()
        self.lib.call("swn_ctx_bytes_allocated", self.handle, C.byref(n))
        return n.value

    def close(self):
        if getattr(self, "handle", None):
            comm = getattr(self, "native_comm", None)
            if comm is not None:
                self.native_comm = None
                comm.close()
            self.lib.call("swn_ctx_destroy", self.handle)
            self.handle = None

    def __del__(self):
        try:
            self.close()
        except Exception:
            pass


_default_ctx = {}


def default_context(device=None, lib=None):
    key = (id(lib) if lib is not None else 0, str(device))
    if key not in _default_ctx:
        _default_ctx[key] = Context(device=device, lib=lib)
    return _default_ctx[key]


class NativeModel:

    def __init__(self, ctx, kind, batch, height, width, is_train=True, dropout=0.5, num_roi=12, body_channels=3,
                 cloth_channels=19, n_layers_D=3, share=None, norm="instance", netG="swapnet"):
        if netG not in NETG_KINDS:
            raise ValueError("Cannot find implementation for " + str(netG))
        if netG != "swapnet" and kind != "texture":
            raise ValueError("netG %s belongs to the texture stage" % netG)
        self.netG = netG
        self.ctx, self.lib, self.kind = ctx, ctx.lib, kind
        self.B, self.H, self.W, self.is_train = batch, height, width, is_train
        self.body_channels, self.cloth_channels = body_channels, cloth_channels
        self.n_layers_D = int(n_layers_D)
        if norm not in NORM_KINDS:
            raise NotImplementedError("normalization layer [%s] is not found" % norm)
        self.norm = norm
        self.share = share
        self.num_roi = share.num_roi if share is not None else int(num_roi)
        if share is not None:
            if share.kind != kind:
                raise ValueError("a sharing model must be of its sharer's kind")
            h = C.c_void_p()
            self.lib.call("swn_model_create_shared", share.handle, batch, height, width, C.byref(h))
            self.is_train, self.body_channels, self.cloth_channels = share.is_train, share.body_channels, share.cloth_channels
            self.n_layers_D, self.out_channels, self.norm = share.n_layers_D, share.out_channels, share.norm
            self.netG = share.netG
            self.handle = h
            self._keep = []
            return
        self.lib.call("swn_ctx_set_patchgan_layers", ctx.handle, self.n_layers_D)
        self.lib.call("swn_ctx_set_patchgan_norm", ctx.handle, NORM_KINDS[norm])
        h = C.c_void_p()
        if kind == "warp":
            self.lib.call("swn_warp_model_create_ex", ctx.handle, batch, height, width, int(is_train),
                          C.c_float(dropout), body_channels, cloth_channels, C.byref(h))
# ... 917 lines not shown
```

Before: 1317 images/sec.

## Fuse strided Winograd filter transform and fp16 panel cut into one pass

Adds a one-pass weight refresh for stride-2 Winograd conv and convT layers. A small amax kernel computes the transformed-filter maximum directly from the packed weights. A panel kernel then applies the filter transform in registers and writes the split fp16 hi/lo GEMM panels directly. This replaces the old path of writing the full fp32 transformed filter U, rereading it and cutting it, and it also drops the U reservation in the gradient buffer. The cost is recomputing the transform twice (amax plus panels), and fp contract is turned off so the fused result matches the old transform bit for bit.

```diff
diff --git a/include/swapnet_hip.h b/include/swapnet_hip.h
--- a/include/swapnet_hip.h
+++ b/include/swapnet_hip.h
@@ -20,6 +20,7 @@
 int swn_ctx_set_overlap(swn_ctx* ctx, int on);
 int swn_ctx_set_patchgan_layers(swn_ctx* ctx, int n_layers);
 int swn_ctx_set_patchgan_norm(swn_ctx* ctx, int kind);
+int swn_ctx_set_refresh_one_pass(swn_ctx* ctx, int on);
 int swn_ctx_sync(swn_ctx* ctx);
 int swn_ctx_bytes_allocated(swn_ctx* ctx, size_t* out);
 
@@ -198,6 +199,8 @@
                       int co, const float* bias, int act, float* y, const int* views, const int32_t* cimap, int cimap_len,
                       int x_is_input, int dgrad_C, int operand_slots, const float* dx_old, const int* pre_range, float* y_fwd,
                       float* y_slot, float* dw_rows, float* x_buf, float* xg_buf, float* y_buf, float* yg_buf);
+int swn_op_refresh_panels(swn_ctx* ctx, int family, int transposed, int mode, const float* packed, int cf, int cc, float* u_scratch,
+                          uint16_t* ref, uint16_t* got, size_t* panel_elems, int* tile);
 int swn_op_adamw(swn_ctx* ctx, float* p, const float* g, float* m, float* v, size_t n, float lr, float b1, float b2,
                  float eps, float wd, int step);
 int swn_op_adabound(swn_ctx* ctx, float* p, const float* g, float* m, float* v, size_t n, float lr, float b1, float b2,
diff --git a/swapnet_amd/_C.py b/swapnet_amd/_C.py
--- a/swapnet_amd/_C.py
+++ b/swapnet_amd/_C.py
@@ -30,6 +30,7 @@
     "swn_ctx_set_overlap": ([_vp, _i], _i),
     "swn_ctx_set_patchgan_layers": ([_vp, _i], _i),
     "swn_ctx_set_patchgan_norm": ([_vp, _i], _i),
+    "swn_ctx_set_refresh_one_pass": ([_vp, _i], _i),
     "swn_ctx_bytes_allocated": ([_vp, C.POINTER(C.c_size_t)], _i),
     "swn_prof_enable": ([_i], _i),
     "swn_prof_reset": ([], _i),
@@ -136,6 +137,7 @@
     "swn_op_norm_act_bwd2": ([_vp, _fp, _fp, _fp, _i, _i, _i, _i, _i, _fp, _fp], _i),
     "swn_op_batch_norm_act_bwd2": ([_vp, _fp, _fp, _fp, _fp, _fp, _i, _i, _i, _i, _i, _fp, _fp, _fp], _i),
     "swn_op_norm_act_dropout": ([_vp, _fp, _fp, _i, _i, _i, _i, _i, _i, _f, C.c_uint64, _fp, _fp, _fp], _i),
+    "swn_op_refresh_panels": ([_vp, _i, _i, _i, _fp, _i, _i, _fp, _vp, _vp, C.POINTER(C.c_size_t), C.POINTER(_i)], _i),
     "swn_op_adamw": ([_vp, _fp, _fp, _fp, _fp, C.c_size_t, _f, _f, _f, _f, _f, _i], _i),
     "swn_op_adabound": ([_vp, _fp, _fp, _fp, _fp, C.c_size_t, _f, _f, _f, _f, _f, _f, _f, _f, _i], _i),
 }
diff --git a/swapnet_amd/csrc/capi.cpp b/swapnet_amd/csrc/capi.cpp
--- a/swapnet_amd/csrc/capi.cpp
+++ b/swapnet_amd/csrc/capi.cpp
@@ -109,6 +109,12 @@
     REQUIRE(ctx, "ctx is NULL");
     REQUIRE(kind >= 0 && kind <= 2, "normalization layer is not found (0 instance, 1 batch, 2 none)");
     ctx->c->patchgan_norm = kind;
+  });
+}
+int swn_ctx_set_refresh_one_pass(swn_ctx* ctx, int on) {
+  return guard([&] {
+    REQUIRE(ctx, "ctx is NULL");
+    ctx->c->refresh_one_pass = on != 0;
   });
 }
 int swn_ctx_sync(swn_ctx* ctx) {
@@ -1495,6 +1501,31 @@
     stream_sync(tmp.s);
   });
 }
+int swn_op_refresh_panels(swn_ctx* ctx, int family, int transposed, int mode, const float* packed, int cf, int cc, float* u_scratch,
+                          uint16_t* ref, uint16_t* got, size_t* panel_elems, int* tile) {
+  return guard([&] {
+    REQUIRE(ctx && packed && panel_elems && tile, "NULL argument");
+    REQUIRE(family == 0, "swn_op_refresh_panels: family 0 (strided Winograd) only");
+    REQUIRE((mode == 0 || mode == 1) && cf > 0 && cc > 0 && cf % 4 == 0 && cc % 4 == 0, "swn_op_refresh_panels: mode 0 / 1, channel counts multiples of 4");
+    WShape w{};
+    w.kind = transposed ? WK_CONVT : WK_CONV; w.KH = w.KW = 4;
+    w.Ci = w.Cip = transposed ? cc : cf; w.Co = w.Npad = transposed ? cf : cc;
+    const int K = mode == 0 ? 4 * cf : cc, N = mode == 0 ? cc : 4 * cf;
+    const int bn = conv_precut_tile(K, N);
+    REQUIRE(bn != 0, "swn_op_refresh_panels: no pre-cut panel for these dimensions");
+    const size_t pe = conv_precut_elems(K, N, bn);
+    *panel_elems = pe; *tile = bn;
+    if (!ref || !got) return;
+    REQUIRE(u_scratch, "swn_op_refresh_panels: u_scratch is NULL");
+    Stream& s = ctx->c->s;
+    const float* wmax = nullptr;
+    wino_s2_filter_transform(s, w, mode, packed, u_scratch);
+    conv_precut(s, u_scratch, K, N, bn, 25, (size_t)K * N, ref, &wmax);
+    const float* umax = wino_s2_filter_amax(s, w, packed);
+    wino_s2_filter_panels(s, w, mode, packed, bn, got, pe, umax);
+    stream_sync(s);
+  });
+}
 int swn_op_adamw(swn_ctx* ctx, float* p, const float* g, float* m, float* v, size_t n, float lr, float b1, float b2,
                  float eps, float wd, int step) {
   return guard([&] {
diff --git a/swapnet_amd/csrc/engine.cpp b/swapnet_amd/csrc/engine.cpp
--- a/swapnet_amd/csrc/engine.cpp
+++ b/swapnet_amd/csrc/engine.cpp
@@ -311,6 +311,13 @@
 }
 bool wino_fwd_takes_pairs(int xC, int Npad) { return wino_precut_tile(xC, Npad) != 0 && conv_fwd_takes_pairs(xC, Npad); }
 
+bool plane_panel_only(size_t T, int K, int N, int tile) {
+  if (!tile || tile != conv_precut_tile(K, N)) return false;
+  const size_t lim = (size_t)1 << 31;
+  return T * (size_t)K * 4 < lim && (size_t)K * N * 4 < lim && (size_t)(K / 16) * ceil_div(N, tile) * 12 * tile * 8 < lim;
+}
+bool refresh_one_pass(const Ctx& c) { return c.refresh_one_pass && is_device_build(); }
+
 bool bias_on_main() { static const bool on = env_on(getenv("SWN_BIAS_MAIN")); return on; }
 }
 
@@ -411,13 +418,14 @@
   const int sP = 25, sTh = ceil_div(y.v.H, 4), sTw = ceil_div(y.v.W, 4), CV = 4 * Cip;
   const size_t sT = (size_t)x.v.N * sTh * sTw;
   const bool want_dx = x.has_grad && y.has_grad;
-  const size_t uf_off = reserve_dg(self, (size_t)sP * CV * Cop);
-  const size_t ut_off = want_dx ? reserve_dg(self, (size_t)sP * Cop * CV) : 0;
+  const int pcf = conv_precut_tile(CV, Cop), pct = want_dx ? conv_precut_tile(Cop, CV) : 0;
+  const bool one_pass = refresh_one_pass(ctx) && plane_panel_only(sT, CV, Cop, pcf) && (!want_dx || plane_panel_only(sT, Cop, CV, pct));
+  const size_t uf_off = one_pass ? 0 : reserve_dg(self, (size_t)sP * CV * Cop);
+  const size_t ut_off = (want_dx && !one_pass) ? reserve_dg(self, (size_t)sP * Cop * CV) : 0;
   float* keepV = (keep_wino_inputs && y.has_grad) ? static_cast<float*>(ctx.alloc(sP * sT * CV * sizeof(float))) : nullptr;
   wsV_need = std::max(wsV_need, sP * sT * (size_t)std::max(CV, Cop));
   wsM_need = std::max(wsM_need, sP * sT * (size_t)std::max(CV, Cop));
   wsU_need = std::max(wsU_need, (size_t)sP * CV * Cop);
-  const int pcf = conv_precut_tile(CV, Cop), pct = want_dx ? conv_precut_tile(Cop, CV) : 0;
   const size_t pcf_bs = pcf ? conv_precut_elems(CV, Cop, pcf) : 0, pct_bs = pct ? conv_precut_elems(Cop, CV, pct) : 0;
   const size_t pcf_off = pcf ? reserve_dgp(pcf_bs * sP) : 0, pct_off = pct ? reserve_dgp(pct_bs * sP) : 0;
   const size_t slV = reserve_slot(), slD = reserve_slot();
@@ -429,6 +437,12 @@
   float* keepdM = (y.has_grad && want_dx && share_dy()) ? static_cast<float*>(ctx.alloc(sP * sT * Cop * sizeof(float))) : nullptr;
   op.repack = [=](Net& n) {
     const ParamDesc& wd = A->params[wi];
+    if (one_pass) {
+      const float* umax = wino_s2_filter_amax(n.ctx.s, wd.ws, A->w + wd.off);
+      wino_s2_filter_panels(n.ctx.s, wd.ws, 0, A->w + wd.off, pcf, n.dgp + pcf_off, pcf_bs, umax);
+      if (want_dx) wino_s2_filter_panels(n.ctx.s, wd.ws, 1, A->w + wd.off, pct, n.dgp + pct_off, pct_bs, umax);
+      return;
+    }
     const float* wmax = nullptr;
     wino_s2_filter_transform(n.ctx.s, wd.ws, 0, A->w + wd.off, n.dg + uf_off);
     if (pcf) conv_precut(n.ctx.s, n.dg + uf_off, CV, Cop, pcf, sP, (size_t)CV * Cop, n.dgp + pcf_off, &wmax);
@@ -443,7 +457,7 @@
     const float* xin = pairV_ok ? n.slot_if_complete(xbase) : nullptr;
     wino_s2_input_transform(n.ctx.s, xv, sTh, sTw, V, n.amax + slV, xin, n.kscale + kV);
     conv_fwd(n.ctx.s, plane_gemm(V, n.wsM, sT, CV, Cop, Co, sP, plane_scale(xin != nullptr, n.kscale + kV, n.amax + slV),
-                                 {n.dg + uf_off, n.dgp + pcf_off, pcf, pcf_bs}));
+                                 {one_pass ? nullptr : n.dg + uf_off, n.dgp + pcf_off, pcf, pcf_bs}));
     wino_output_transform(n.ctx.s, 4, 2, n.wsM, Cop, sTh, sTw, bi >= 0 ? A->w + A->params[bi].off : nullptr, actf, yv, Co, 0);
   };
   Var scratch;
@@ -475,7 +489,7 @@
     if (!dx_now) return;
     float* dMx = shared ? keepdM : n.wsV;
     if (!shared) wino_dy_transform(n.ctx.s, 4, 2, dY, sTh, sTw, dMx, n.amax + slD, din, n.kscale + kD);
-    conv_fwd(n.ctx.s, plane_gemm(dMx, n.wsM, sT, Cop, CV, CV, sP, dMs, {n.dg + ut_off, n.dgp + pct_off, pct, pct_bs}));
+    conv_fwd(n.ctx.s, plane_gemm(dMx, n.wsM, sT, Cop, CV, CV, sP, dMs, {one_pass ? nullptr : n.dg + ut_off, n.dgp + pct_off, pct, pct_bs}));
     wino_s2_input_adjoint(n.ctx.s, n.wsM, Cip, sTh, sTw, xgv, nullptr, me.acc.empty() ? 0 : me.acc[0]);
   };
 }
@@ -847,13 +861,14 @@
   const int sP = 25, sTh = ceil_div(x.v.H, 4), sTw = ceil_div(x.v.W, 4), CV = 4 * Cop;
   const size_t sT = (size_t)x.v.N * sTh * sTw;
   const bool want_dx = x.has_grad && y.has_grad;
-  const size_t ut_off = reserve_dg(self, (size_t)sP * Cip * CV);
-  const size_t uf_off = want_dx ? reserve_dg(self, (size_t)sP * CV * Cip) : 0;
+  const int pct = conv_precut_tile(Cip, CV), pcf = want_dx ? conv_precut_tile(CV, Cip) : 0;
+  const bool one_pass = refresh_one_pass(ctx) && plane_panel_only(sT, Cip, CV, pct) && (!want_dx || plane_panel_only(sT, CV, Cip, pcf));
+  const size_t ut_off = one_pass ? 0 : reserve_dg(self, (size_t)sP * Cip * CV);
+  const size_t uf_off = (want_dx && !one_pass) ? reserve_dg(self, (size_t)sP * CV * Cip) : 0;
   float* keepM = (keep_wino_inputs && y.has_grad) ? static_cast<float*>(ctx.alloc(sP * sT * Cip * sizeof(float))) : nullptr;
   wsV_need = std::max(wsV_need, sP * sT * (size_t)std::max(CV, Cip));
   wsM_need = std::max(wsM_need, sP * sT * (size_t)std::max(CV, Cip));
   wsU_need = std::max(wsU_need, (size_t)sP * CV * Cip);
-  const int pct = conv_precut_tile(Cip, CV), pcf = want_dx ? conv_precut_tile(CV, Cip) : 0;
   const size_t pct_bs = pct ? conv_precut_elems(Cip, CV, pct) : 0, pcf_bs = pcf ? conv_precut_elems(CV, Cip, pcf) : 0;
   const size_t pct_off = pct ? reserve_dgp(pct_bs * sP) : 0, pcf_off = pcf ? reserve_dgp(pcf_bs * sP) : 0;
   const size_t slM = reserve_slot(), slV = reserve_slot();
@@ -864,6 +879,12 @@
   float* keepVg = (y.has_grad && want_dx && share_dy()) ? static_cast<float*>(ctx.alloc(sP * sT * CV * sizeof(float))) : nullptr;
   op.repack = [=](Net& n) {
     const ParamDesc& wd = A->params[wi];
+    if (one_pass) {
+      const float* umax = wino_s2_filter_amax(n.ctx.s, wd.ws, A->w + wd.off);
+      wino_s2_filter_panels(n.ctx.s, wd.ws, 1, A->w + wd.off, pct, n.dgp + pct_off, pct_bs, umax);
+      if (want_dx) wino_s2_filter_panels(n.ctx.s, wd.ws, 0, A->w + wd.off, pcf, n.dgp + pcf_off, pcf_bs, umax);
+      return;
+    }
     wino_s2_filter_transform(n.ctx.s, wd.ws, 1, A->w + wd.off, n.dg + ut_off);
     const float* wmax = nullptr;
     if (pct) conv_precut(n.ctx.s, n.dg + ut_off, Cip, CV, pct, sP, (size_t)Cip * CV, n.dgp + pct_off, &wmax);
@@ -878,7 +899,7 @@
     const float* xin = pairM_ok ? n.slot_if_complete(xbase) : nullptr;
     wino_dy_transform(n.ctx.s, 4, 2, xv, sTh, sTw, dM, n.amax + slM, xin, n.kscale + kM);
     conv_fwd(n.ctx.s, plane_gemm(dM, n.wsM, sT, Cip, CV, CV, sP, plane_scale(xin != nullptr, n.kscale + kM, n.amax + slM),
-                                 {n.dg + ut_off, n.dgp + pct_off, pct, pct_bs}));
+                                 {one_pass ? nullptr : n.dg + ut_off, n.dgp + pct_off, pct, pct_bs}));
     wino_s2_input_adjoint(n.ctx.s, n.wsM, Cop, sTh, sTw, yv, bi >= 0 ? A->w + A->params[bi].off : nullptr, 0);
   };
   if (want_dx) op.grad_targets.push_back(x);
@@ -905,7 +926,7 @@
     if (!dx_now) return;
     float* Vx = shared ? keepVg : n.wsV;
     if (!shared) wino_s2_input_transform(n.ctx.s, ygv, sTh, sTw, Vx, n.amax + slV, din, n.kscale + kVg);
-    conv_fwd(n.ctx.s, plane_gemm(Vx, n.wsM, sT, CV, Cip, Cip, sP, Vs, {n.dg + uf_off, n.dgp + pcf_off, pcf, pcf_bs}));
+    conv_fwd(n.ctx.s, plane_gemm(Vx, n.wsM, sT, CV, Cip, Cip, sP, Vs, {one_pass ? nullptr : n.dg + uf_off, n.dgp + pcf_off, pcf, pcf_bs}));
     wino_output_transform(n.ctx.s, 4, 2, n.wsM, Cip, sTh, sTw, nullptr, ACT_NONE, xgv, Cip, me.acc.empty() ? 0 : me.acc[0]);
   };
 }
@@ -1964,6 +1985,12 @@
   g.bound = 2 + (size_t)(g.chunks - 1) * png_chunk_cap((size_t)g.chunk_bytes) + png_chunk_cap((size_t)g.last_bytes) + 4;
   return g;
 }
+__attribute__((weak)) const float* wino_s2_filter_amax(Stream&, const WShape&, const float*) {
+  throw Error(1, "wino_s2_filter_amax: the one-pass operand refresh is not implemented on the host simulator (HIP kernel only)");
+}
+__attribute__((weak)) void wino_s2_filter_panels(Stream&, const WShape&, int, const float*, int, uint16_t*, size_t, const float*) {
+  throw Error(1, "wino_s2_filter_panels: the one-pass operand refresh is not implemented on the host simulator (HIP kernel only)");
+}
 __attribute__((weak)) void png_encode(Stream&, const PngEncodeArgs&) {
   throw Error(1, "png_encode: PNG encoding is not implemented on the host simulator (HIP kernel only)");
 }
diff --git a/swapnet_amd/csrc/engine.h b/swapnet_amd/csrc/engine.h
--- a/swapnet_amd/csrc/engine.h
+++ b/swapnet_amd/csrc/engine.h
@@ -45,6 +45,7 @@
   void all_reduce_sum(Stream& on, float* buf, size_t count);
   int patchgan_layers = 3;
   int patchgan_norm = 0;
+  bool refresh_one_pass = true;
   explicit Ctx(void* stream, size_t ws_bytes);
   explicit Ctx(const Stream& shared);
   bool owns_ws = true;
diff --git a/swapnet_amd/csrc/ops.h b/swapnet_amd/csrc/ops.h
--- a/swapnet_amd/csrc/ops.h
+++ b/swapnet_amd/csrc/ops.h
@@ -138,6 +138,9 @@
 void wino_s2_input_adjoint(Stream& s, float* dV, int Cf, int Th, int Tw, const TView& fine, const float* bias, int accumulate);
 void wino_s2_filter_transform(Stream& s, const WShape& w, int mode, const float* packed, float* U);
 void wino_s2_filter_grad(Stream& s, const WShape& w, const float* dU, float* dpacked);
+const float* wino_s2_filter_amax(Stream& s, const WShape& w, const float* packed);
+void wino_s2_filter_panels(Stream& s, const WShape& w, int mode, const float* packed, int bn, uint16_t* out, size_t panel_elems,
+                           const float* wamax);
 void wino_filter_grad(Stream& s, int m, int r, const WShape& w, const float* dU, float* dpacked);
 
 struct NormActArgs {
diff --git a/swapnet_amd/csrc/wino.hip b/swapnet_amd/csrc/wino.hip
--- a/swapnet_amd/csrc/wino.hip
+++ b/swapnet_amd/csrc/wino.hip
@@ -710,6 +710,15 @@
   return (size_t)(a * 2 + b) * 4 * w.Cip * w.Npad + ((size_t)(dy * 2 + dx) * w.Cip + cc) * w.Npad + cf;
 }
 
+__device__ __forceinline__ float s2_gg(int r, float g0, float g1) {
+#pragma clang fp contract(off)
+  return F42::G[r][0] * g0 + F42::G[r][1] * g1;
+}
+__device__ __forceinline__ float s2_ggt(float t0, float t1, int j) {
+#pragma clang fp contract(off)
+  return t0 * F42::G[j][0] + t1 * F42::G[j][1];
+}
+
 __global__ __launch_bounds__(256) void wino_s2_filter_kernel(WShape w, int mode, int Cf, int Cc, const float* packed, float* U) {
   constexpr int A = 5;
   const size_t total = (size_t)Cf * Cc;
@@ -729,12 +738,12 @@
 #pragma unroll
     for (int r = 0; r < A; ++r)
 #pragma unroll
-      for (int b = 0; b < 2; ++b) tt[r][b] = F42::G[r][0] * g[0][b] + F42::G[r][1] * g[1][b];
+      for (int b = 0; b < 2; ++b) tt[r][b] = s2_gg(r, g[0][b], g[1][b]);
     const size_t o = mode == 0 ? ((size_t)(q * Cf + cf) * Cc + cc) : ((size_t)cc * 4 * Cf + q * Cf + cf);
 #pragma unroll
     for (int a = 0; a < A; ++a)
 #pragma unroll
-      for (int j = 0; j < A; ++j) U[(size_t)(a * A + j) * plane + o] = tt[a][0] * F42::G[j][0] + tt[a][1] * F42::G[j][1];
+      for (int j = 0; j < A; ++j) U[(size_t)(a * A + j) * plane + o] = s2_ggt(tt[a][0], tt[a][1], j);
   }
 }
 
@@ -890,6 +899,125 @@
 }
 
 
+__global__ __launch_bounds__(256) void s2_filter_amax_kernel(WShape w, int Cf, int Cc, const float* packed, float* part) {
+  constexpr int A = 5;
+  const size_t total = (size_t)Cf * Cc;
+  const bool conv = w.kind == WK_CONV;
+  float m = 0.f;
+  for (size_t i = (size_t)blockIdx.x * 256 + threadIdx.x; i < total; i += (size_t)256 * 256) {
+    const int cf = conv ? (int)(i / Cc) : (int)(i % Cf), cc = conv ? (int)(i % Cc) : (int)(i / Cf);
+#pragma unroll
+    for (int q = 0; q < 4; ++q) {
+      const int s = q >> 1, t = q & 1;
+      float g[2][2];
+#pragma unroll
+      for (int a = 0; a < 2; ++a)
+#pragma unroll
+        for (int b = 0; b < 2; ++b) g[a][b] = packed[s2_widx(w, 2 * a + s, 2 * b + t, cf, cc)];
+#pragma unroll
+      for (int a = 0; a < A; ++a) {
+        const float t0 = s2_gg(a, g[0][0], g[1][0]), t1 = s2_gg(a, g[0][1], g[1][1]);
+#pragma unroll
+        for (int j = 0; j < A; ++j) m = fmaxf(m, fabsf(s2_ggt(t0, t1, j)));
+      }
+    }
+  }
+#pragma unroll
+  for (int o = 32; o; o >>= 1) m = fmaxf(m, __shfl_xor(m, o));
+  __shared__ float red[4];
+  if ((threadIdx.x & 63) == 0) red[threadIdx.x >> 6] = m;
+  __syncthreads();
+  if (threadIdx.x == 0) part[blockIdx.x] = fmaxf(fmaxf(red[0], red[1]), fmaxf(red[2], red[3]));
+}
+
+__device__ __forceinline__ void s2_cut8_store(const float (&u)[8], float sb, wu32x4* o, size_t e0, size_t plane_stride, bool low_plane) {
+  unsigned hi[4], lo[4];
+#pragma unroll
+  for (int j = 0; j < 4; ++j) {
+    const float x0 = u[2 * j] * sb, x1 = u[2 * j + 1] * sb;
+    const wf16x2 hh = wf16x2{(_Float16)x0, (_Float16)x1};
+    hi[j] = __builtin_bit_cast(unsigned, hh) | ((__float_as_uint(x0) >> 16) & 0x8000u) | (__float_as_uint(x1) & 0x80000000u);
+    const float h0 = (float)hh[0] + 0.f, h1 = (float)hh[1] + 0.f;
+    lo[j] = __builtin_bit_cast(unsigned, wf16x2{(_Float16)(x0 - h0), (_Float16)(x1 - h1)});
+  }
+  o[e0] = wu32x4{hi[0], hi[1], hi[2], hi[3]};
+  if (low_plane) o[e0 + plane_stride] = wu32x4{lo[0], lo[1], lo[2], lo[3]};
+}
+
+__global__ __launch_bounds__(256) void s2_panel_kernel(WShape w, int mode, int Cf, int Cc, int BN, const float* packed, unsigned short* out,
+                                                       size_t panel_elems, const float* wamax, int planes) {
+  constexpr int A = 5;
+  const int K = mode == 0 ? 4 * Cf : Cc, Nn = mode == 0 ? Cc : 4 * Cf;
+  const int NBc = BN / 32, tiles_n = (Nn + BN - 1) / BN;
+  const size_t total = (size_t)(K / 8) * tiles_n * BN;
+  const size_t i = (size_t)blockIdx.x * 256 + threadIdx.x;
+  const int PL = planes;
+  const int kB = wino_scale_exp(wamax, threadIdx.x & 63, 10);
+  if (i >= total) return;
+  const int nl = (int)(i % BN); const size_t qi = i / BN;
+  const int tn = (int)(qi % tiles_n), kq = (int)(qi / tiles_n);
+  const int n = tn * BN + nl;
+  const int pos = (nl % NBc) * 32 + nl / NBc;
+  const bool valid = n < Nn;
+  float g[8][2][2];
+#pragma unroll
+  for (int kk = 0; kk < 8; ++kk)
+#pragma unroll
+    for (int a = 0; a < 2; ++a)
+#pragma unroll
+      for (int b = 0; b < 2; ++b) g[kk][a][b] = 0.f;
+  if (valid) {
+    const bool kcontig = (mode == 1) == (w.kind == WK_CONV) && (mode == 1 || Cf % 8 == 0);
+    if (kcontig) {
+      const int k0 = kq * 8;
+      const int q = mode == 0 ? k0 / Cf : n / Cf;
+      const int cf = mode == 0 ? k0 - q * Cf : n - q * Cf, cc = mode == 0 ? n : k0;
+      const int s = q >> 1, t = q & 1;
+#pragma unroll
+      for (int a = 0; a < 2; ++a)
+#pragma unroll
+        for (int b = 0; b < 2; ++b) {
+          const float4* src = reinterpret_cast<const float4*>(packed + s2_widx(w, 2 * a + s, 2 * b + t, cf, cc));
+          const float4 v0 = src[0], v1 = src[1];
+          g[0][a][b] = v0.x; g[1][a][b] = v0.y; g[2][a][b] = v0.z; g[3][a][b] = v0.w;
+          g[4][a][b] = v1.x; g[5][a][b] = v1.y; g[6][a][b] = v1.z; g[7][a][b] = v1.w;
+        }
+    } else {
+#pragma unroll
+      for (int kk = 0; kk < 8; ++kk) {
+        const int k = kq * 8 + kk;
+        const int q = mode == 0 ? k / Cf : n / Cf;
+        const int cf = mode == 0 ? k - q * Cf : n - q * Cf, cc = mode == 0 ? n : k;
+        const int s = q >> 1, t = q & 1;
+#pragma unroll
+        for (int a = 0; a < 2; ++a)
+#pragma unroll
+          for (int b = 0; b < 2; ++b) g[kk][a][b] = packed[s2_widx(w, 2 * a + s, 2 * b + t, cf, cc)];
+      }
+    }
+  }
+  const size_t e0 = ((((size_t)(kq >> 1) * tiles_n + tn) * 2 + (kq & 1)) * PL) * BN + pos;
+  const float sb = __uint_as_float((unsigned)(127 + kB) << 23);
+#pragma unroll
+  for (int a = 0; a < A; ++a) {
+    float tt[8][2];
+#pragma unroll
+    for (int kk = 0; kk < 8; ++kk)
+#pragma unroll
+      for (int b = 0; b < 2; ++b) tt[kk][b] = s2_gg(a, g[kk][0][b], g[kk][1][b]);
+#pragma unroll
+    for (int j = 0; j < A; ++j) {
+      float u[8];
+#pragma unroll
+      for (int kk = 0; kk < 8; ++kk) u[kk] = valid ? s2_ggt(tt[kk][0], tt[kk][1], j) : 0.f;
+      unsigned short* panel = out + (size_t)(a * A + j) * panel_elems;
+      s2_cut8_store(u, sb, reinterpret_cast<wu32x4*>(panel), e0, (size_t)BN, PL == 2);
+      if (i == 0) *reinterpret_cast<int*>(panel + (size_t)(K / 16) * tiles_n * 2 * PL * BN * 8) = kB;
+    }
+  }
+}
+
+
 __device__ __forceinline__ size_t tailw_fold_off(int Cip, int Npad, int ph) {
   const int pre = ph == 0 ? 0 : (ph == 1 ? 4 : (ph == 2 ? 10 : 16));
   return (size_t)pre * Cip * Npad;
@@ -1061,6 +1189,8 @@
 inline unsigned wgrid(size_t total) { return (unsigned)std::min<size_t>(std::max<size_t>((total + 255) / 256, 1), 256 * 32); }
 
 }
+
+float* ws_amax(Stream& s, int which);
 
 static int variant(int m, int r) {
   if (m == 2 && r == 3) return 0;
@@ -1232,6 +1362,28 @@
   hipLaunchKernelGGL(wino_s2_filter_grad_kernel, dim3((unsigned)(((size_t)Cf * Cc + 255) / 256)), dim3(256), 0, hs(s), w, Cf, Cc, dU, dpacked);
   check_launch("wino_s2_filter_grad");
 }
+const float* wino_s2_filter_amax(Stream& s, const WShape& w, const float* packed) {
+  int Cf, Cc;
+  s2_dims(w, Cf, Cc);
+  float* part = ws_amax(s, 1);
+  hipLaunchKernelGGL(s2_filter_amax_kernel, dim3(256), dim3(256), 0, hs(s), w, Cf, Cc, packed, part);
+  check_launch("wino_s2_filter_amax");
+  return part;
+}
+void wino_s2_filter_panels(Stream& s, const WShape& w, int mode, const float* packed, int bn, uint16_t* out, size_t panel_elems,
+                           const float* wamax) {
+  int Cf, Cc;
+  s2_dims(w, Cf, Cc);
+  if (mode != 0 && mode != 1) throw Error(1, "wino_s2_filter_panels: mode 0 or 1");
+  const int K = mode == 0 ? 4 * Cf : Cc, Nn = mode == 0 ? Cc : 4 * Cf;
+  if (K % 16 || Cf % 4 || (bn != 64 && bn != 128 && bn != 192)) throw Error(1, "wino_s2_filter_panels: K must be a multiple of 16, tile 64, 128 or 192");
+  if (panel_elems != conv_precut_elems(K, Nn, bn)) throw Error(1, "wino_s2_filter_panels: panel stride does not match conv_precut_elems");
+  if (!wamax || ((uintptr_t)packed & 15)) throw Error(1, "wino_s2_filter_panels: needs the partial maxima of wino_s2_filter_amax and 16-byte aligned weights");
+  const size_t total = (size_t)(K / 8) * ((Nn + bn - 1) / bn) * bn;
+  hipLaunchKernelGGL(s2_panel_kernel, dim3((unsigned)((total + 255) / 256)), dim3(256), 0, hs(s), w, mode, Cf, Cc, bn, packed, out, panel_elems,
+                     wamax, conv_precut_planes());
+  check_launch("wino_s2_filter_panels");
+}
 void wino_input_adjoint(Stream& s, int m, int r, float* dV, int C, int pad, int pad_mode, int Th, int Tw, const TView& dx,
                         int accumulate) {
   const int v = variant(m, r);
diff --git a/swapnet_amd/engine.py b/swapnet_amd/engine.py
--- a/swapnet_amd/engine.py
+++ b/swapnet_amd/engine.py
@@ -74,6 +74,9 @@
 
     def set_overlap(self, on):
         self.lib.call("swn_ctx_set_overlap", self.handle, int(bool(on)))
+
+    def set_refresh_one_pass(self, on):
+        self.lib.call("swn_ctx_set_refresh_one_pass", self.handle, int(bool(on)))
 
     def sync(self):
         self.lib.call("swn_ctx_sync", self.handle)
```

Result: no change. 1330 images/sec, median of 6 (+1.0%).
